# ZhuoQiuMcgill/ReinforcementLearning4MeshGeneration

Measured on AMD Instinct MI355X. Metric: env-steps/sec at N_envs=4096 per GPU, boundary() domain, 1 MI355X, higher is better.
Workload: dtype f64

## Files before the change

reinforcementlearning4meshgeneration_amd/csrc/meshenv_eval.h:

```cpp
#pragma once

#include "meshenv_quality.h"

namespace meshenv {

constexpr int kEvalWaves = 8;

struct EvalTallyArgs {
    int n, step;
    const double *reward;
    const uint8_t *done, *complete;
    const LastEpisode *last_ep;
    const int32_t *target, *offset;
    int32_t *count, *length, *seen;
    double *ret, *ret_raw;
    int32_t *short_envs;
    int32_t *ep_env, *ep_domain, *ep_step, *ep_length, *ep_flags, *ep_n_elem, *ep_archive;
    double *ep_return, *ep_return_raw, *ep_quality;
};

__global__ void __launch_bounds__(64) k_eval_begin(DevState S, EvalTallyArgs A)
{
    const int lane = lane_id(), env = blockIdx.x * 64 + lane;
    bool wants = false;
    if (env < A.n) {
        A.count[env] = 0;
        A.length[env] = 0;
        A.ret[env] = 0.0;
        A.ret_raw[env] = 0.0;
        A.seen[env] = A.last_ep ? A.last_ep[env].episodes : 0;
        wants = A.target[env] > 0;
    }
    const unsigned long long m = __ballot(wants);
    if (lane == 0 && m) atomicAdd(A.short_envs, (int)__popcll(m));
}

__global__ void __launch_bounds__(64 * kEvalWaves) k_eval_tally(DevState S, EvalTallyArgs A)
{
    __shared__ int s_slot[64];
    __shared__ unsigned long long s_rec, s_scored;
    const int lane = lane_id(), wave = uniform_i32(threadIdx.x >> 6);
    const int base = blockIdx.x * 64, env = base + lane;
    if (wave == 0) {
        const bool live = env < A.n;
        bool rec = false, archived = false, reached = false;
        int slot = 0;
        if (live) {
            const double r = A.reward[env];
            const int len = A.length[env] + 1;
            const double ret = A.ret[env] + (double)(float)r;
            const double raw = A.ret_raw[env] + r;
            const LastEpisode le = A.last_ep ? A.last_ep[env] : LastEpisode{0, 0, 0, 0};
            const int seen = A.seen[env];
            if (A.last_ep && le.episodes != seen) A.seen[env] = le.episodes;
            if (A.done[env]) {
                archived = A.last_ep && le.episodes != seen;
                const int cnt = A.count[env], tgt = A.target[env];
                if (cnt < tgt) {
                    rec = true;
                    slot = A.offset[env] + cnt;
                    A.ep_env[slot] = env;
                    A.ep_domain[slot] = S.scal[env].dom;
                    A.ep_step[slot] = A.step;
                    A.ep_length[slot] = len;
                    A.ep_return[slot] = ret;
                    A.ep_return_raw[slot] = raw;
                    A.ep_flags[slot] = (A.complete[env] ? 1 : 0) | (archived ? (le.flags & 2) : 0);
                    A.ep_n_elem[slot] = A.last_ep ? (archived ? le.n_elem : 0) : -1;
                    if (A.ep_archive) A.ep_archive[slot] = archived ? le.episodes : 0;
                    A.count[env] = cnt + 1;
                    reached = cnt + 1 == tgt;
                }
                A.length[env] = 0;
                A.ret[env] = 0.0;
                A.ret_raw[env] = 0.0;
            } else {
                A.length[env] = len;
                A.ret[env] = ret;
                A.ret_raw[env] = raw;
            }
        }
        s_slot[lane] = slot;
        const unsigned long long rec_mask = __ballot(rec), scored_mask = __ballot(rec && archived);
        const unsigned long long reached_mask = __ballot(reached);
        if (lane == 0 && reached_mask) atomicSub(A.short_envs, (int)__popcll(reached_mask));
        if (lane == 0) {
            s_rec = rec_mask;
            s_scored = scored_mask;
        }
    }
    if (!A.ep_quality) return;
    __syncthreads();
    const unsigned long long rec = s_rec, scored = s_scored;
    unsigned long long todo = ((unsigned long long)(unsigned)uniform_i32((int)(rec >> 32)) << 32) |
                              (unsigned)uniform_i32((int)(unsigned)rec);
    if (!todo) return;
    const DevCold cold = *S.cold;
    for (int k = 0; todo; k++) {
        const int l = __builtin_ctzll(todo);
        todo &= todo - 1;
        if (k % kEvalWaves != wave) continue;
        double *row = A.ep_quality + (size_t)uniform_i32(s_slot[l]) * 4 * kQualityDim;
        if ((scored >> l) & 1) env_quality(S, S.scal[base + l], cold, base + l, 1, nullptr, row, nullptr);
        else if (lane < 4 * kQualityDim) row[lane] = 0.0;
    }
}

}
```

reinforcementlearning4meshgeneration_amd/csrc/meshenv_hip.hip:

```cpp
#include "../../include/meshenv.h"
#include "../../include/meshenv_optim.h"

#include <hip/hip_runtime.h>
#include <link.h>

#include <cmath>
#include <cstdio>
#include <cstdlib>
#include <cstring>
#include <mutex>
#include <string>
#include <vector>

#include "meshenv_actor.h"
#include "meshenv_domgen.h"
#include "meshenv_kernels.h"
#include "meshenv_quality.h"
#include "meshenv_smooth.h"
#include "meshenv_samples.h"
#include "meshenv_fused.h"
#include "meshenv_policy.h"
#include "meshenv_gae.h"
#include "meshenv_eval.h"
#include "meshenv_replay.h"
// ... 410 lines not shown
    }
    CREATE_HIP(upload_atan_state());

    {
        int n_cu = 256;
        CREATE_HIP(hipDeviceGetAttribute(&n_cu, hipDeviceAttributeMultiprocessorCount, device));
        if (n_cu <= 0) n_cu = 256;
        h->n_cu = n_cu;
        int G = 1;
        const char *force = getenv("MESHENV_GROUP");
        int want = 1;
        if (force) want = atoi(force);
        else if (n_envs <= n_cu * 16) {
            int g = 1;
            while (g * 2 <= n_envs / n_cu && g * 2 <= 16) g *= 2;
            want = g >= 8 ? g : 1;
        }
        for (int g : {16, 8})
            if (g <= want && group_lds_bytes(cap, g) <= 150 * 1024) { G = g; break; }
        if (!force && (G < 8 || n_envs > n_cu * G)) G = 1;
        if (G == 1 && want == 16 && n_envs <= n_cu * 16 && group_lds_bytes(cap, 16) > 150 * 1024) {
            std::vector<int2> pack((size_t)n_envs);
            size_t worst = 0;
            for (int w0 = 0; w0 < n_envs; w0 += 16) {
                size_t off = 0;
                for (int e = w0; e < w0 + 16 && e < n_envs; e++) {
                    const int d = env_domain_host[e];
                    const int n0 = dom_offsets_host[d + 1] - dom_offsets_host[d];
                    const int cap_e = (n0 + 15) / 16 * 16;
                    pack[(size_t)e] = make_int2((int)off, cap_e);
                    off += lds_bytes_for(cap_e);
                }
                worst = off > worst ? off : worst;
            }
            worst = (worst + 31) / 32 * 32;
            if (worst + 16 * sizeof(Handoff) <= (size_t)kLdsCap) {
                G = 16;
                h->env_lds_host.swap(pack);
                h->ho_off = (int)worst;
            }
        }
        MeshEnvParams def;
        meshenv_default_params(&def);
        h->default_params = prm.radius == def.radius && prm.max_ref_angle == def.max_ref_angle && prm.key_lambda == def.key_lambda &&
                            prm.min_degree == def.min_degree && prm.max_degree == def.max_degree &&
                            prm.same_point_eps == def.same_point_eps && prm.ray_length == def.ray_length;
        if (!h->default_params) G = 1;
        if (!h->default_params) h->env_lds_host.clear();
        h->group = G;
        h->group_lds = h->env_lds_host.empty() ? group_lds_bytes(cap, G) : (size_t)h->ho_off + 16 * sizeof(Handoff);
        {
            const char *lz = getenv("MESHENV_LAZY");
            const bool lazy = lz ? atoi(lz) != 0 : n_envs >= 8192;
            const char *lt = getenv("MESHENV_LIGHT");
            const bool light = lt ? atoi(lt) != 0 : (lazy && n_envs >= 16384);
            h->stage_bits = (lazy ? 2 : 0) | (light ? 4 : 0);
        }
        if (G > 1 && h->group_lds > 64 * 1024) {
            const bool ragged = !h->env_lds_host.empty();
            const void *fn = ragged ? (const void *)k_step_group<16, true, true>
                             : G == 16 ? (const void *)k_step_group<16, true> : (const void *)k_step_group<8, true>;
            if (!ragged && cap <= 64) fn = G == 16 ? (const void *)k_step_group<16, true, false, true> : (const void *)k_step_group<8, true, false, true>;
            CREATE_HIP(hipFuncSetAttribute(fn, hipFuncAttributeMaxDynamicSharedMemorySize, kLdsCap));
        }
    }

    DevState &S = h->S;
    S.n_domains = n_domains;
    S.n_envs = n_envs;
    S.prm.radius = prm.radius;
    S.prm.max_ref_angle = prm.max_ref_angle;
    S.prm.w0 = prm.key_lambda;
    S.prm.w1 = 1 - prm.key_lambda;
    S.prm.min_degree = prm.min_degree;
    S.prm.max_degree = prm.max_degree;
    S.prm.same_eps = prm.same_point_eps;
    S.prm.ray_length = prm.ray_length;
    S.prm.fail_limit = prm.fail_limit;
    S.prm.log_cap = prm.log_capacity;

    const int total_dom = dom_offsets_host[n_domains];
    h->dom_off_host.assign(dom_offsets_host, dom_offsets_host + n_domains + 1);
    h->env_dom_host.assign(env_domain_host, env_domain_host + n_envs);
    const size_t total_env = (size_t)n_envs * (size_t)cap;
    S.cap = cap;

    double2 *d_dom_xy = nullptr;
    DevCold &K = h->cold;
    std::memset(&K, 0, sizeof(K));
    CREATE_TRY(dev_alloc(h, &S.dom, (size_t)n_domains));
    CREATE_TRY(dev_alloc(h, &d_dom_xy, (size_t)total_dom));
    CREATE_TRY(dev_alloc(h, &K.dom_key, (size_t)total_dom));
    CREATE_TRY(dev_alloc(h, &K.dom_stamp, (size_t)total_dom));
    CREATE_TRY(dev_alloc(h, &K.dom_obs, (size_t)n_domains * kObsDim));
    CREATE_TRY(dev_alloc(h, &S.ring_xy, total_env));
    CREATE_TRY(dev_alloc(h, &S.ring_id, total_env));
    CREATE_TRY(dev_alloc(h, &S.ring_key, total_env));
    CREATE_TRY(dev_alloc(h, &S.ring_stamp, total_env));
    CREATE_TRY(dev_alloc(h, &S.scal, (size_t)n_envs));
    CREATE_TRY(dev_alloc(h, &S.cnt, (size_t)n_envs));
    CREATE_TRY(dev_alloc(h, &S.obs_cache, (size_t)n_envs * kObsDim));
    if (!h->env_lds_host.empty()) {
        CREATE_TRY(dev_alloc(h, &h->env_lds, (size_t)n_envs));
        CREATE_HIP(hipMemcpy(h->env_lds, h->env_lds_host.data(), sizeof(int2) * (size_t)n_envs, hipMemcpyHostToDevice));
    }
    if (prm.log_capacity > 0) {
        CREATE_TRY(dev_alloc(h, &K.log_quads, (size_t)n_envs * 2 * prm.log_capacity * 4));
        CREATE_TRY(dev_alloc(h, &K.log_vxy, (size_t)n_envs * 2 * prm.log_capacity));
        CREATE_TRY(dev_alloc(h, &K.last_ep, (size_t)n_envs));
        CREATE_HIP(hipMemsetAsync(K.last_ep, 0, sizeof(LastEpisode) * (size_t)n_envs, h->stream));
    }
    K.dom_xy = d_dom_xy;
    {
        DevCold *cold_dev = nullptr;
        CREATE_TRY(dev_alloc(h, &cold_dev, (size_t)1));
        CREATE_HIP(hipMemcpy(cold_dev, &K, sizeof(DevCold), hipMemcpyHostToDevice));
        S.cold = cold_dev;
    }
#ifdef MESHENV_STAMPS
    CREATE_TRY(dev_alloc(h, &S.dbg, (size_t)n_envs * 16));
#endif

    std::vector<EnvScalars> sc((size_t)n_envs);
    std::memset(sc.data(), 0, sc.size() * sizeof(EnvScalars));
    for (int e = 0; e < n_envs; e++) sc[e].dom = env_domain_host[e];

    if (!gen) {
        std::vector<DomConst> dc((size_t)n_domains);
        std::memset(dc.data(), 0, dc.size() * sizeof(DomConst));
        for (int d = 0; d < n_domains; d++) {
            dc[d].orig_area = dom_consts_host[3 * d];
            dc[d].min_area = dom_consts_host[3 * d + 1] * dom_consts_host[3 * d + 1];
            dc[d].crit_area = dom_consts_host[3 * d + 2] * dom_consts_host[3 * d + 2];
            dc[d].off = dom_offsets_host[d];
            dc[d].n0 = dom_offsets_host[d + 1] - dom_offsets_host[d];
            dc[d].ref = -1;
        }
        CREATE_HIP(hipMemcpy(S.dom, dc.data(), sizeof(DomConst) * (size_t)n_domains, hipMemcpyHostToDevice));
        CREATE_HIP(hipMemcpy(d_dom_xy, dom_xy_host, sizeof(double2) * (size_t)total_dom, hipMemcpyHostToDevice));
    } else {
        int32_t *d_off = nullptr;
        int *d_err = nullptr;
        CREATE_TRY(dev_alloc(h, &d_off, (size_t)n_domains + 1));
        CREATE_TRY(dev_alloc(h, &d_err, (size_t)1));
        CREATE_HIP(hipMemcpy(d_off, dom_offsets_host, sizeof(int32_t) * ((size_t)n_domains + 1), hipMemcpyHostToDevice));
        CREATE_HIP(hipMemset(d_err, 0, sizeof(int)));
        if (gen->density_mode)
            hipLaunchKernelGGL(k_gen_rings_density, dim3(n_domains), dim3(64), 0, h->stream, *gen, n_domains, (const int32_t *)d_off, d_dom_xy, d_err);
        else
            hipLaunchKernelGGL(k_gen_rings, dim3(n_domains), dim3(64), 0, h->stream, *gen, n_domains, (const int32_t *)d_off, d_dom_xy, d_err);
        CREATE_HIP(hipGetLastError());
        hipLaunchKernelGGL(k_dom_consts, dim3(n_domains), dim3(64), sizeof(double2) * (size_t)max_ring, h->stream, n_domains,
                           (const int32_t *)d_off, (const double2 *)d_dom_xy, S.dom);
        CREATE_HIP(hipGetLastError());
        int err = 0;
        CREATE_HIP(hipMemcpy(&err, d_err, sizeof(int), hipMemcpyDeviceToHost));
        if (err) {
            g_create_error = "meshenv_create_random: a ring could not be generated on the device (fewer than 5 distinct pixels, or a length mismatch between the two passes)";
            meshenv_destroy(h);
            return MESHENV_E_STATE;
        }
    }
    CREATE_HIP(hipMemcpy(S.scal, sc.data(), sizeof(EnvScalars) * (size_t)n_envs, hipMemcpyHostToDevice));
    CREATE_HIP(hipMemset(S.ring_xy, 0, sizeof(double2) * total_env));
    CREATE_HIP(hipMemset(S.ring_id, 0, sizeof(int32_t) * total_env));
    CREATE_HIP(hipMemset(S.ring_key, 0, sizeof(double) * total_env));
    CREATE_HIP(hipMemset(S.ring_stamp, 0, sizeof(int32_t) * total_env));

    hipLaunchKernelGGL(k_init_domains, dim3(n_domains), dim3(64), lds, h->stream, S, cap);
    CREATE_HIP(hipGetLastError());
    hipLaunchKernelGGL(k_reset, dim3(n_envs), dim3(64), lds, h->stream, S, cap, (const uint8_t *)nullptr, (float *)nullptr, 1, 0ULL,
                       0, (int32_t *)nullptr, (int32_t *)nullptr);
    CREATE_HIP(hipGetLastError());
    CREATE_HIP(hipStreamSynchronize(h->stream));
#undef CREATE_TRY
#undef CREATE_HIP
    *out = h;
    return MESHENV_OK;
}

extern "C" {

int meshenv_create(int device, int n_domains, const int32_t *dom_offsets_host, const double *dom_xy_host,
                   const double *dom_consts_host, int n_envs, const int32_t *env_domain_host,
                   const MeshEnvParams *params, void *stream, MeshEnv **out)
{
    return create_impl(device, n_domains, dom_offsets_host, dom_xy_host, dom_consts_host, n_envs, env_domain_host, params,
                       stream, nullptr, out);
}

static void edge_direction(double dx, double dy, bool integer, double *cs)
{
    volatile double ny = (integer && dy == 0) ? 0.0 : -dy, x = dx;
    const double theta = -std::atan2(ny, x);
    volatile double angle = std::copysign(1.0, theta) >= 0 ? theta : 2 * 3.141592653589793 + theta;
    cs[0] = std::cos(angle);
    cs[1] = std::sin(angle);
}

static int create_random_impl(const char *fn, int device, int n_envs, GenParams gp, const uint64_t *seeds_host,
                              const MeshEnvParams *params, void *stream, MeshEnv **out, uint8_t *raises_host)
{
    int ndev = 0;
    if (hipGetDeviceCount(&ndev) != hipSuccess || ndev <= 0) {
        g_create_error = std::string(fn) + ": no HIP device available (this library has no CPU fallback)";
        return MESHENV_E_HIP;
    }
    if (device < 0 || device >= ndev) return fail_arg(nullptr, "meshenv_create_random: device index out of range");
    std::vector<int32_t> offs((size_t)n_envs + 1, 0), env_dom((size_t)n_envs);
    DeviceGuard guard(device);
    if (guard.err != hipSuccess) { g_create_error = std::string(fn) + ": hipSetDevice failed"; return MESHENV_E_HIP; }
    int32_t *d_cnt = nullptr;
    int *d_err = nullptr;
    unsigned long long *d_seeds = nullptr;
    double2 *d_tab = nullptr;
    unsigned char *d_raises = nullptr;
    auto cleanup = [&]() {
        if (d_cnt) (void)hipFree(d_cnt);
        if (d_err) (void)hipFree(d_err);
        if (d_seeds) (void)hipFree(d_seeds);
        if (d_tab) (void)hipFree(d_tab);
        if (d_raises) (void)hipFree(d_raises);
    };
    bool ok = hipMalloc((void **)&d_cnt, sizeof(int32_t) * (size_t)n_envs) == hipSuccess &&
              hipMalloc((void **)&d_err, sizeof(int)) == hipSuccess && hipMemset(d_err, 0, sizeof(int)) == hipSuccess;
    if (ok && seeds_host) {
        ok = hipMalloc((void **)&d_seeds, sizeof(unsigned long long) * (size_t)n_envs) == hipSuccess &&
             hipMemcpy(d_seeds, seeds_host, sizeof(unsigned long long) * (size_t)n_envs, hipMemcpyHostToDevice) == hipSuccess;
        gp.seeds = d_seeds;
    }
    if (ok && gp.density_mode) {
        const int R = (int)std::ceil(4 * gp.ave_radius) + 1, W = 2 * R + 1;
        std::vector<double> tab((size_t)W * W * 2);
        for (int dx = -R; dx <= R; dx++)
            for (int dy = -R; dy <= R; dy++) edge_direction((double)dx, (double)dy, true, &tab[((size_t)(dx + R) * W + (dy + R)) * 2]);
        ok = hipMalloc((void **)&d_tab, sizeof(double2) * (size_t)W * W) == hipSuccess &&
             hipMemcpy(d_tab, tab.data(), sizeof(double) * tab.size(), hipMemcpyHostToDevice) == hipSuccess &&
             hipMalloc((void **)&d_raises, (size_t)n_envs) == hipSuccess && hipMemset(d_raises, 0, (size_t)n_envs) == hipSuccess;
        gp.dir_tab = d_tab;
        gp.dir_r = R;
        gp.raises = d_raises;
    }
    int err = 0;
    if (ok) {
        if (gp.density_mode) hipLaunchKernelGGL(k_gen_count_density, dim3(n_envs), dim3(64), 0, (hipStream_t)stream, gp, n_envs, d_cnt, d_err);
        else hipLaunchKernelGGL(k_gen_count, dim3(n_envs), dim3(64), 0, (hipStream_t)stream, gp, n_envs, d_cnt, d_err);
        ok = hipGetLastError() == hipSuccess && hipStreamSynchronize((hipStream_t)stream) == hipSuccess &&
             hipMemcpy(offs.data() + 1, d_cnt, sizeof(int32_t) * (size_t)n_envs, hipMemcpyDeviceToHost) == hipSuccess &&
             hipMemcpy(&err, d_err, sizeof(int), hipMemcpyDeviceToHost) == hipSuccess;
    }
// ... 427 lines not shown
    const size_t lds = smooth_lds_bytes(h->cap, log_cap), lds_front = smooth_front_lds_bytes(h->cap, log_cap);
    if (lds > 160 * 1024 || (!interior && lds_front > 160 * 1024) || h->cap + log_cap > 65535)
        return fail_arg(h, "meshenv_smooth: ring stride + log_capacity too large for the smoother's LDS (16 B per ring slot + 60 B per logged vertex; front smoother 51 B per vertex)");
    MESHENV_ON_DEVICE(h);
    {
        const int rc = ensure_smooth_state(h);
        if (rc != MESHENV_OK) return rc;
    }
    int32_t *sw = sweeps_dev ? sweeps_dev : h->smooth_sweeps;
    if (!interior) return launch_full_smoothing(h, mask_dev, iteration, is_static, sw, diff_dev, obs_dev);
    const dim3 grid(h->n_envs), block(64);
    hipLaunchKernelGGL(k_smooth_interior, grid, block, lds, h->stream, h->S, h->cap, which, mask_dev, (const int32_t *)nullptr,
                       iteration, sw, diff_dev);
    HIP_TRY(h, hipGetLastError());
    if (which) return MESHENV_OK;
    hipLaunchKernelGGL(k_rebuild_candidates<0>, grid, block, h->lds, h->stream, h->S, h->cap, mask_dev, sw, h->pend, h->pend_obs,
                       (float *)nullptr, libm_ref(h));
    HIP_TRY(h, hipGetLastError());
    h->reselect_pending = true;
    return MESHENV_OK;
}

int meshenv_smooth_final(MeshEnv *h, int which, const uint8_t *mask_dev, int iteration, double lr_1, double lr_2,
                         int32_t *sweeps_dev, double *diff_dev)
{
    if (!h || (which != 0 && which != 1)) return MESHENV_E_ARG;
    if (iteration < 0) return fail_arg(h, "meshenv_smooth_final: iteration must be >= 0");
    const int log_cap = h->S.prm.log_cap;
    if (log_cap <= 0) {
        h->err = "meshenv_smooth_final: handle was created with log_capacity = 0 (the mesh graph is rebuilt from the element log)";
        return MESHENV_E_STATE;
    }
    const size_t lds = smooth_final_lds_bytes(h->cap, log_cap);
    if (lds > 160 * 1024 || h->cap + log_cap > 65535)
        return fail_arg(h, "meshenv_smooth_final: ring stride + log_capacity too large for the smoother's LDS (51 B per vertex)");
    MESHENV_ON_DEVICE(h);
    if (!h->smooth_final_ready) {
        HIP_TRY(h, hipFuncSetAttribute((const void *)k_smooth_final, hipFuncAttributeMaxDynamicSharedMemorySize, 160 * 1024));
        h->smooth_final_ready = true;
    }
    hipLaunchKernelGGL(k_smooth_final, dim3(h->n_envs), dim3(64), lds, h->stream, h->S, h->cap, which, mask_dev, iteration, lr_1,
                       lr_2, sweeps_dev, diff_dev);
    HIP_TRY(h, hipGetLastError());
    return MESHENV_OK;
}

int meshenv_get_not_valid(MeshEnv *h, int env, double *xy_host, int cap_points, int32_t *count)
{
    if (!h || !count) return MESHENV_E_ARG;
    if (env < 0 || env >= h->n_envs) {
        h->err = "meshenv_get_not_valid: env out of range";
        return MESHENV_E_RANGE;
    }
    *count = 0;
    if (!h->move_ready) return MESHENV_OK;
    MESHENV_ON_DEVICE(h);
    HIP_TRY(h, hipStreamSynchronize(h->stream));
    int32_t n = 0;
    HIP_TRY(h, hipMemcpy(&n, h->nv_count + env, sizeof(n), hipMemcpyDeviceToHost));
    *count = n;
    if (xy_host && n > 0) {
        const int m = n < cap_points ? n : cap_points;
        HIP_TRY(h, hipMemcpy(xy_host, h->nv_xy + (size_t)env * h->cap, sizeof(double2) * (size_t)m, hipMemcpyDeviceToHost));
    }
    return MESHENV_OK;
}

int meshenv_get_not_valid_ids(MeshEnv *h, int env, int32_t *ids_host, int cap_ids, int32_t *count, int32_t *last_host)
{
    if (!h || !count) return MESHENV_E_ARG;
    if (env < 0 || env >= h->n_envs) {
        h->err = "meshenv_get_not_valid_ids: env out of range";
        return MESHENV_E_RANGE;
    }
    *count = 0;
    if (last_host) last_host[0] = last_host[1] = last_host[2] = last_host[3] = 0;
    if (!h->move_ready) return MESHENV_OK;
    MESHENV_ON_DEVICE(h);
    HIP_TRY(h, hipStreamSynchronize(h->stream));
    int32_t n = 0, meta[kNvMeta];
    HIP_TRY(h, hipMemcpy(&n, h->nv_count + env, sizeof(n), hipMemcpyDeviceToHost));
    HIP_TRY(h, hipMemcpy(meta, h->nv_meta + (size_t)env * kNvMeta, sizeof(meta), hipMemcpyDeviceToHost));
    EnvScalars s;
    HIP_TRY(h, hipMemcpy(&s, h->S.scal + env, sizeof(s), hipMemcpyDeviceToHost));
    const int n0 = h->dom_off_host[s.dom + 1] - h->dom_off_host[s.dom];
    auto gid = [n0](int32_t g) { return (g & kNewBit) ? n0 + (g & ~kNewBit) : g; };
    *count = n;
    if (ids_host && n > 0) {
        const int m = n < cap_ids ? n : cap_ids;
        HIP_TRY(h, hipMemcpy(ids_host, h->nv_gid + (size_t)env * h->cap, sizeof(int32_t) * (size_t)m, hipMemcpyDeviceToHost));
        for (int i = 0; i < m; i++) ids_host[i] = gid(ids_host[i]);
    }
    if (last_host) {
        last_host[0] = gid(meta[1]); last_host[1] = gid(meta[2]); last_host[2] = meta[3];
        last_host[3] = meta[4] == meta[0] ? 1 : 0;
    }
    return MESHENV_OK;
}

static int launch_step(MeshEnv *h, int n_steps, const float *actions_dev, float *obs_dev, double *reward_dev,
                       uint8_t *done_dev, uint8_t *complete_dev, float *terminal_obs_dev, int auto_reset)
{
    if (!h) return MESHENV_E_ARG;
    if (!actions_dev || !obs_dev || !reward_dev || !done_dev || !complete_dev) return fail_arg(h, "meshenv_step: null device pointer");
    if (n_steps <= 0) return fail_arg(h, "meshenv_rollout: n_steps must be positive");
    if (n_steps > 1 && h->reselect_pending) {
        h->err = "meshenv_rollout: the first step after meshenv_smooth must be a meshenv_step (it commits the re-selection "
                 "the candidate rebuild parked, include/meshenv.h)";
        return MESHENV_E_STATE;
    }
    MESHENV_ON_DEVICE(h);
    const size_t slot = (size_t)(h->ev_count % MESHENV_TIMING_POOL);
    const long long pos = h->timing > 0 ? (h->launch_count++ % (2LL * h->timing)) : -1;
    if (pos == 0) HIP_TRY(h, hipEventRecord(h->ev[2 * slot], h->stream));
    if (n_steps == 1 && h->group > 1 && !h->front_moved) {
        const int G = h->group;
        const dim3 grid((h->n_envs + G - 1) / G), block(64 * G);
        GroupArgs A;
        A.S = h->S;
        A.outs.obs_out = obs_dev; A.outs.reward = reward_dev; A.outs.done = done_dev; A.outs.complete = complete_dev;
        A.outs.term_obs = terminal_obs_dev;
        A.actions = actions_dev;
        A.step0 = (unsigned long long)h->steps_done;
        A.cap = h->cap;
        A.auto_reset = auto_reset;
        A.env_lds = h->env_lds;
        A.ho_off = h->ho_off;
        A.pad = 0;
        if (h->env_lds) hipLaunchKernelGGL((k_step_group<16, true, true>), grid, block, h->group_lds, h->stream, A);
        else if (h->cap <= 64 && G == 16) hipLaunchKernelGGL((k_step_group<16, true, false, true>), grid, block, h->group_lds, h->stream, A);
        else if (h->cap <= 64) hipLaunchKernelGGL((k_step_group<8, true, false, true>), grid, block, h->group_lds, h->stream, A);
        else if (G == 16) hipLaunchKernelGGL((k_step_group<16, true>), grid, block, h->group_lds, h->stream, A);
        else hipLaunchKernelGGL((k_step_group<8, true>), grid, block, h->group_lds, h->stream, A);
    } else {
        const dim3 grid(h->n_envs), block(64);
#define MESHENV_LAUNCH_STEP(MULTI, DEF)                                                                                      \
    do {                                                                                                                     \
        KStepArgs ka;                                                                                                        \
        ka.S = h->S; ka.cap = h->cap; ka.n_steps = n_steps; ka.actions = actions_dev; ka.obs_out = obs_dev;                  \
        ka.reward = reward_dev; ka.done = done_dev; ka.complete = complete_dev; ka.term_obs = terminal_obs_dev;              \
        ka.auto_reset = auto_reset; ka.step0 = (unsigned long long)h->steps_done;                                            \
        if (h->front_moved) hipLaunchKernelGGL((k_step<MULTI, DEF, true>), grid, block, h->lds, h->stream, ka);              \
        else if (DEF && !MULTI && (h->stage_bits & 2) && h->cap <= 64)                                                       \
            hipLaunchKernelGGL((k_step<false, DEF, false, DEF, DEF>), grid, block, h->lds, h->stream, ka);                   \
        else if (DEF && !MULTI && (h->stage_bits & 2))                                                                       \
            hipLaunchKernelGGL((k_step<false, DEF, false, false, DEF>), grid, block, h->lds, h->stream, ka);                 \
        else if (DEF && h->cap <= 64) hipLaunchKernelGGL((k_step<MULTI, DEF, false, DEF>), grid, block, h->lds, h->stream, ka); \
        else hipLaunchKernelGGL((k_step<MULTI, DEF>), grid, block, h->lds, h->stream, ka);                                   \
    } while (0)
        if (n_steps == 1) {
            auto_reset = (auto_reset ? 1 : 0) | h->stage_bits;
            if (h->default_params) MESHENV_LAUNCH_STEP(false, true);
            else MESHENV_LAUNCH_STEP(false, false);
        } else {
            if (h->default_params) MESHENV_LAUNCH_STEP(true, true);
            else MESHENV_LAUNCH_STEP(true, false);
        }
#undef MESHENV_LAUNCH_STEP
    }
    HIP_TRY(h, hipGetLastError());
    if (h->reselect_pending) {
        hipLaunchKernelGGL(k_apply_reselect, dim3(h->n_envs), dim3(64), 0, h->stream, h->S, h->pend, h->pend_obs, obs_dev);
        HIP_TRY(h, hipGetLastError());
        h->reselect_pending = false;
    }
    h->steps_done += (uint64_t)n_steps;
    if (pos >= 0 && pos == h->timing - 1) {
        HIP_TRY(h, hipEventRecord(h->ev[2 * slot + 1], h->stream));
        h->ev_count += 1;
    }
    return MESHENV_OK;
}

int meshenv_step(MeshEnv *h, const float *actions_dev, float *obs_dev, double *reward_dev, uint8_t *done_dev,
                 uint8_t *complete_dev, float *terminal_obs_dev, int auto_reset)
{
    return launch_step(h, 1, actions_dev, obs_dev, reward_dev, done_dev, complete_dev, terminal_obs_dev, auto_reset);
}

int meshenv_rollout(MeshEnv *h, int n_steps, const float *actions_dev, float *obs_dev, double *reward_dev,
                    uint8_t *done_dev, uint8_t *complete_dev, int auto_reset)
{
    return launch_step(h, n_steps, actions_dev, obs_dev, reward_dev, done_dev, complete_dev, nullptr, auto_reset);
}

__global__ void k_status(DevState S, uint8_t *out)
{
    const int e = blockIdx.x * blockDim.x + threadIdx.x;
    if (e < S.n_envs) out[e] = (uint8_t)(S.scal[e].status & 3);
}

int meshenv_get_status(MeshEnv *h, uint8_t *status_dev)
{
    if (!h || !status_dev) return MESHENV_E_ARG;
    MESHENV_ON_DEVICE(h);
    hipLaunchKernelGGL(k_status, dim3((h->n_envs + 255) / 256), dim3(256), 0, h->stream, h->S, status_dev);
    HIP_TRY(h, hipGetLastError());
    return MESHENV_OK;
}

int meshenv_get_state(MeshEnv *h, int env, int32_t *ring_ids_host, double *ring_xy_host, double *cand_key_host,
                      int32_t *cand_stamp_host, int32_t *scalars_host, double *fscalars_host)
{
    if (!h) return MESHENV_E_ARG;
    if (env < 0 || env >= h->n_envs) {
        h->err = "meshenv_get_state: env out of range";
        return MESHENV_E_RANGE;
    }
    MESHENV_ON_DEVICE(h);
    HIP_TRY(h, hipStreamSynchronize(h->stream));
    EnvScalars s;
    HIP_TRY(h, hipMemcpy(&s, h->S.scal + env, sizeof(s), hipMemcpyDeviceToHost));
    const size_t off = (size_t)env * (size_t)h->cap;
    const int n0 = h->dom_off_host[s.dom + 1] - h->dom_off_host[s.dom];
    const int n = s.n;
    if (ring_ids_host) {
        HIP_TRY(h, hipMemcpy(ring_ids_host, h->S.ring_id + off, sizeof(int32_t) * n, hipMemcpyDeviceToHost));
        for (int i = 0; i < n; i++)
            if (ring_ids_host[i] & kNewBit) ring_ids_host[i] = n0 + (ring_ids_host[i] & ~kNewBit);
    }
    if (ring_xy_host) HIP_TRY(h, hipMemcpy(ring_xy_host, h->S.ring_xy + off, sizeof(double2) * n, hipMemcpyDeviceToHost));
    if (cand_stamp_host || cand_key_host) {
        std::vector<int32_t> st((size_t)n);
        std::vector<double> ky((size_t)n);
        HIP_TRY(h, hipMemcpy(st.data(), h->S.ring_stamp + off, sizeof(int32_t) * n, hipMemcpyDeviceToHost));
        HIP_TRY(h, hipMemcpy(ky.data(), h->S.ring_key + off, sizeof(double) * n, hipMemcpyDeviceToHost));
        for (int i = 0; i < n; i++) {
            if (cand_stamp_host) cand_stamp_host[i] = st[i];
            if (cand_key_host) cand_key_host[i] = st[i] == kNotCand ? NAN : ky[i];
        }
    }
    if (scalars_host) {
        scalars_host[0] = s.n;
        scalars_host[1] = s.ref;
        scalars_host[2] = s.n_elem;
        scalars_host[3] = s.failed;
        scalars_host[4] = n0 + s.n_new;
        scalars_host[5] = s.status & 3;
        scalars_host[6] = s.dom;
        scalars_host[7] = n0;
    }
    if (fscalars_host) {
        fscalars_host[0] = s.area;
        fscalars_host[1] = s.bl;
    }
    return MESHENV_OK;
}

static int fetch_elements(MeshEnv *h, const char *fn, int which, int env, int32_t *quads_host, int cap_elems,
                          double *vertex_xy_host, int cap_verts, int32_t *n_elem, int32_t *n_vert, int32_t *flags,
                          int32_t *episodes)
{
    if (!h || !n_elem || !n_vert) return MESHENV_E_ARG;
    if (env < 0 || env >= h->n_envs) {
        h->err = std::string(fn) + ": env out of range";
        return MESHENV_E_RANGE;
    }
    const int cap = h->S.prm.log_cap;
    if (cap <= 0) {
        h->err = std::string(fn) + ": handle was created with log_capacity = 0";
        return MESHENV_E_STATE;
    }
    MESHENV_ON_DEVICE(h);
    HIP_TRY(h, hipStreamSynchronize(h->stream));
    EnvScalars s;
    HIP_TRY(h, hipMemcpy(&s, h->S.scal + env, sizeof(s), hipMemcpyDeviceToHost));
    int half = (s.status >> 4) & 1, ne = s.n_elem, nnew = s.n_new;
    if (which) {
        LastEpisode le;
        HIP_TRY(h, hipMemcpy(&le, h->cold.last_ep + env, sizeof(le), hipMemcpyDeviceToHost));
        half ^= 1; ne = le.n_elem; nnew = le.n_new;
        if (flags) *flags = le.flags;
        if (episodes) *episodes = le.episodes;
    }
    const int d = s.dom;
    const int n0 = h->dom_off_host[d + 1] - h->dom_off_host[d];
    ne = ne < cap ? ne : cap;
    nnew = nnew < cap ? nnew : cap;
    if (ne > cap_elems) ne = cap_elems;
    int nv = n0 + nnew;
    if (nv > cap_verts) nv = cap_verts;
    const size_t base = ((size_t)env * 2 + half) * cap;
    if (quads_host && ne > 0) {
        HIP_TRY(h, hipMemcpy(quads_host, h->cold.log_quads + base * 4, sizeof(int32_t) * 4 * (size_t)ne, hipMemcpyDeviceToHost));
        for (int i = 0; i < 4 * ne; i++)
            if (quads_host[i] & kNewBit) quads_host[i] = n0 + (quads_host[i] & ~kNewBit);
    }
    if (vertex_xy_host && nv > 0) {
        const int first = nv < n0 ? nv : n0;
        HIP_TRY(h, hipMemcpy(vertex_xy_host, h->cold.dom_xy + h->dom_off_host[d], sizeof(double2) * (size_t)first, hipMemcpyDeviceToHost));
        if (nv > n0)
            HIP_TRY(h, hipMemcpy(vertex_xy_host + 2 * (size_t)n0, h->cold.log_vxy + base, sizeof(double2) * (size_t)(nv - n0), hipMemcpyDeviceToHost));
    }
    *n_elem = ne;
    *n_vert = nv;
    return MESHENV_OK;
}

int meshenv_get_elements(MeshEnv *h, int env, int32_t *quads_host, int cap_elems, double *vertex_xy_host,
                         int cap_verts, int32_t *n_elem, int32_t *n_vert)
{
    return fetch_elements(h, "meshenv_get_elements", 0, env, quads_host, cap_elems, vertex_xy_host, cap_verts, n_elem,
                          n_vert, nullptr, nullptr);
}

int meshenv_get_last_episode(MeshEnv *h, int env, int32_t *quads_host, int cap_elems, double *vertex_xy_host,
                             int cap_verts, int32_t *n_elem, int32_t *n_vert, int32_t *flags, int32_t *episodes)
{
    return fetch_elements(h, "meshenv_get_last_episode", 1, env, quads_host, cap_elems, vertex_xy_host, cap_verts,
                          n_elem, n_vert, flags, episodes);
}

int meshenv_element_quality(MeshEnv *h, int which, double *elem_dev, double *stats_dev, int32_t *count_dev)
{
    if (!h || (which != 0 && which != 1)) return MESHENV_E_ARG;
    if (h->S.prm.log_cap <= 0) {
        h->err = "meshenv_element_quality: handle was created with log_capacity = 0";
        return MESHENV_E_STATE;
    }
    MESHENV_ON_DEVICE(h);
    hipLaunchKernelGGL(k_element_quality, dim3(h->n_envs), dim3(64), 0, h->stream, h->S, which, elem_dev, stats_dev,
                       count_dev);
    HIP_TRY(h, hipGetLastError());
    return MESHENV_OK;
}

int meshenv_quad_quality(MeshEnv *h, int n, const double *quad_xy_dev, int index, double *out_dev)
{
    if (!h || n < 0 || (n > 0 && (!quad_xy_dev || !out_dev))) return MESHENV_E_ARG;
    if (!(index == 0 || index == 1 || index == 3 || index == 4 || index == 5))
        return fail_arg(h, "meshenv_quad_quality: index must be 0, 1, 3, 4 or 5 (2 and 6 add the boundary term of the extraction "
                           "step: that value is the step's reward)");
    if (n == 0) return MESHENV_OK;
    MESHENV_ON_DEVICE(h);
    hipLaunchKernelGGL(k_quad_quality, dim3((n + 63) / 64), dim3(64), 0, h->stream, n,
                       reinterpret_cast<const double2 *>(quad_xy_dev), index, out_dev);
    HIP_TRY(h, hipGetLastError());
    return MESHENV_OK;
}

int meshenv_counters(MeshEnv *h, uint64_t *out_host)
{
    if (!h || !out_host) return MESHENV_E_ARG;
    MESHENV_ON_DEVICE(h);
    HIP_TRY(h, hipStreamSynchronize(h->stream));
    std::vector<EnvCounters> c((size_t)h->n_envs);
    std::vector<EnvScalars> sc((size_t)h->n_envs);
    HIP_TRY(h, hipMemcpy(c.data(), h->S.cnt, sizeof(EnvCounters) * (size_t)h->n_envs, hipMemcpyDeviceToHost));
    HIP_TRY(h, hipMemcpy(sc.data(), h->S.scal, sizeof(EnvScalars) * (size_t)h->n_envs, hipMemcpyDeviceToHost));
    uint64_t a = h->steps_done * (uint64_t)h->n_envs, b = 0, s = 0, sv = 0;
    for (int e = 0; e < h->n_envs; e++) {
        const EnvCounters &k = c[(size_t)e];
        b += k.valid;
        s += k.sum_n + (uint64_t)sc[(size_t)e].n * (h->steps_done - k.last_change);
        sv += k.sum_n_valid;
    }
    out_host[0] = a;
    out_host[1] = b;
    out_host[2] = s;
    out_host[3] = sv;
    return MESHENV_OK;
}

#ifdef MESHENV_STAMPS
int meshenv_debug_raw_counters(MeshEnv *h, uint64_t *out_host)
{
    if (!h || !out_host) return MESHENV_E_ARG;
    HIP_TRY(h, hipStreamSynchronize(h->stream));
    HIP_TRY(h, hipMemcpy(out_host, h->S.cnt, sizeof(EnvCounters) * (size_t)h->n_envs, hipMemcpyDeviceToHost));
    return MESHENV_OK;
}
int meshenv_debug_stamps(MeshEnv *h, uint64_t *out_host)
{
    if (!h || !out_host) return MESHENV_E_ARG;
    HIP_TRY(h, hipStreamSynchronize(h->stream));
    HIP_TRY(h, hipMemcpy(out_host, h->S.dbg, sizeof(uint64_t) * 16 * (size_t)h->n_envs, hipMemcpyDeviceToHost));
    return MESHENV_OK;
}
#endif

__global__ void k_selftest(int what, int n, const double *in, double *out, int libm_exact)
{
    const int i = blockIdx.x * blockDim.x + threadIdx.x;
    if (i >= n) return;
    if (what == 0) out[i] = round4_py(in[i]);
    else if (what == 1) out[i] = round4_np(in[i]);
    else if (what == 2) out[i] = cw(mkp(in[6 * i], in[6 * i + 1]), mkp(in[6 * i + 2], in[6 * i + 3]), mkp(in[6 * i + 4], in[6 * i + 5]));
    else if (what == 3) out[i] = is_cross(mkp(in[8 * i], in[8 * i + 1]), mkp(in[8 * i + 2], in[8 * i + 3]), mkp(in[8 * i + 4], in[8 * i + 5]),
                                          mkp(in[8 * i + 6], in[8 * i + 7])) ? 1.0 : 0.0;
    else if (what == 4) out[i] = (sin_rounds_to_zero(in[2 * i], in[2 * i + 1]) ? 1.0 : 0.0) + (sin_rounds_to_zero_exact(in[2 * i], in[2 * i + 1]) ? 2.0 : 0.0);
    else if (what == 5) out[i] = (double)round4_npf((float)in[i]);
    else if (what == 6) out[i] = dist(mkp(in[4 * i], in[4 * i + 1]), mkp(in[4 * i + 2], in[4 * i + 3]));
    else if (what == 7) out[i] = (sqrt_pos(in[i]) == sqrt(in[i])) ? 1.0 : 0.0;
    else if (what == 8) {
        bool ne;
        const double f = cw_fast(in[2 * i], in[2 * i + 1], ne);
        const double e = cw_exact(in[2 * i], in[2 * i + 1]);
        out[i] = ne ? 1.0 : ((f == e && signbit(f) == signbit(e)) ? 0.0 : 2.0);
    } else if (what == 9 || what == 10) {
        const double *q = in + 9 * (size_t)i;
        FrontState f;
        f.coord = nullptr; f.adj = nullptr; f.deg = nullptr; f.ringu = nullptr; f.n = 0; f.n0 = 0; f.raised = 0; f.tab = nullptr; f.exact = libm_exact != 0;
        const P2 v = mkp(q[1], q[2]), a = mkp(q[3], q[4]), b = mkp(q[5], q[6]);
        const int which = (int)q[0];
        P2 r;
        if (which == 0) r = middle_vertex(f, v, a, b, q[7]);
        else if (which == 1) r = side_vertex(f, v, a, b, q[7], q[8], false);
        else if (which == 2) r = indention_vertex(f, v, a, b, q[7], q[8], false);
        else {
            const double2 e = estimate_4th_vertex(make_double2(v.x, v.y), make_double2(a.x, a.y), make_double2(b.x, b.y), q[7], q[8] >= 0, q[8]);
            r = mkp(e.x, e.y);
        }
        out[i] = f.raised ? __builtin_nan("") : (what == 9 ? r.x : r.y);
    } else if (what == 11) out[i] = pow2_glibc(in[i]);
    else if (what == 12) out[i] = cw_exact(in[2 * i], in[2 * i + 1]);
    else if (what == 13) {
        bool ok;
        const double t = atan2_glibc(in[2 * i], in[2 * i + 1], g_atan_cij, ok);
        out[i] = ok ? t : __builtin_nan("");
    } else if (what == 14) out[i] = atan2_cr(in[2 * i], in[2 * i + 1]);
    else if (what == 15) out[i] = sincos_small_nc(in[i]).s;
    else if (what == 16) out[i] = sincos_small_nc(in[i]).c;
    else if (what == 17) {
        const double *q = in + 7 * (size_t)i;
        const P2 ref = mkp(q[0], q[1]);
        const double tl = q[4];
        const double ux = (ref.x + q[2]) - ref.x, uy = (ref.y + q[3]) - ref.y;
        const P2 v = mkp(q[5], ref.y - 1), b = mkp(q[6], ref.y + 1);
        const double W = slab_half_width(tl);
        const double slab_lo = ref.x - W, slab_hi = ref.x + W;
        double s;
        out[i] = (slab_keeps(slab_lo, slab_hi, v.x, b.x) ? 1.0 : 0.0) + (bisector_hits(ref, ux, uy, v, b, s) ? 2.0 : 0.0) +
                 (dist(ref, v) < tl ? 4.0 : 0.0);
    } else if (what == 18) {
        const double *q = in + 7 * (size_t)i;
        const P2 p = mkp(q[0], q[1]), vi = mkp(q[2], q[3]), vm = mkp(q[4], q[5]), far = mkp(q[6], q[1]);
        out[i] = (pip_filter_usable(fabs(q[6] - p.x)) && pip_edge_clear(p, vi, vm) ? 1.0 : 0.0) + (straddle(p, far, vi, vm) && straddle(vi, vm, p, far) ? 2.0 : 0.0);
    } else if (what == 19) {
        const double *q = in + 9 * (size_t)i;
        P2 m[4];
        for (int k = 0; k < 4; k++) m[k] = mkp(q[2 * k], q[2 * k + 1]);
        double rec[kQualityDim];
        element_quality(m, rec);
        double r = __builtin_nan("");
        for (int k = 0; k < kQualityDim; k++) r = q[8] == (double)k ? rec[k] : r;
        out[i] = r;
    }
}

int meshenv_selftest(int device, int what, int n, int in_per_item, const double *in_host, double *out_host)
{
    if (n <= 0 || !in_host || !out_host || in_per_item <= 0) return MESHENV_E_ARG;
// ... 1329 lines not shown
```

reinforcementlearning4meshgeneration_amd/csrc/meshenv_kernels.h:

```cpp
#pragma once

#include "meshenv_geom.h"
#include "meshenv_libm.h"
#include "meshenv_state.h"

namespace meshenv {

constexpr int kStNoReference = 1;
constexpr int kStLogOverflow = 2;
constexpr int kStRm1Bad = 4, kStRp1Bad = 8;
constexpr int kNvMeta = 8;
constexpr int kStLogHalf = 16;

#ifdef MESHENV_STAMPS
#define MESHENV_STAMP(c, k) do { if ((c).lane == 0) (c).sc->stamps[k] = __builtin_amdgcn_s_memrealtime(); } while (0)
#else
#define MESHENV_STAMP(c, k) do { } while (0)
#endif

struct Scratch {
    double2 q[4];
    double ang[4];
    double tmp[16];
    double tmp2[8];
    float robs[18];
    int ipad[2];
    unsigned long long red[6];
#ifdef MESHENV_STAMPS
    unsigned long long stamps[16];
#endif
};

struct Ctx {
    double2 *xy;
    double *key;
    int32_t *stamp;
    int32_t *id;
    double *ang_ord;
    int32_t *list;
    Scratch *sc;
    int lane, env;
    size_t base;
    int n, ref, n_elem, failed, n_new, counter, status, dom;
    double bl, area, ct, st;
    bool ring_dirty;
    bool tie = false;
    float obs;
};

__device__ __forceinline__ P2 ldp(const Ctx &c, int i)
{
    const double2 v = c.xy[i];
    return mkp(v.x, v.y);
}

__device__ __forceinline__ void wave_sync()
{
    __builtin_amdgcn_fence(__ATOMIC_ACQ_REL, "wavefront");
    __builtin_amdgcn_wave_barrier();
}

__device__ __forceinline__ int spin_until_nonzero(volatile int *w)
{
    int v = *w;
    for (int it = 0; v == 0 && it < (1 << 22); it++) {
        __builtin_amdgcn_s_sleep(1);
        v = *w;
    }
    return v;
}

__device__ __forceinline__ int wrapi(int i, int n)
{
    const unsigned a = (unsigned)i, b = (unsigned)(i + n), c = (unsigned)(i - n);
    const unsigned m = a < b ? a : b;
    return (int)(m < c ? m : c);
}

__host__ __device__ __forceinline__ size_t lds_bytes_for(int cap)
{
    return ((size_t)cap * (sizeof(double2) + 2 * sizeof(double) + 3 * sizeof(int32_t)) + sizeof(Scratch) + 64 + 15) / 16 * 16;
}

__device__ __forceinline__ void carve_lds(Ctx &c, void *smem, int cap)
{
    c.xy = (double2 *)smem;
    c.key = (double *)(c.xy + cap);
    c.ang_ord = c.key + cap;
    c.stamp = (int32_t *)(c.ang_ord + cap);
    c.id = c.stamp + cap;
    c.list = c.id + cap;
    c.sc = (Scratch *)(c.list + cap);
}


struct EnvLoad {
    EnvScalars s;
    double2 v_xy, w_xy;
    double v_key, w_key;
    int v_id, v_st, w_id, w_st;
    float obs;
};

__device__ __forceinline__ EnvLoad load_env_issue(const DevState &S, int env, const bool with_keys = true)
{
    EnvLoad L;
    const int lane = lane_id();
    const size_t base = (size_t)env * S.cap;
    L.s = S.scal[env];
    const int first = S.cap < 64 ? S.cap : 64;
    const double2 *gxy = S.ring_xy + base;
    const int32_t *gid = S.ring_id + base;
    const double *gkey = S.ring_key + base;
    const int32_t *gst = S.ring_stamp + base;
    const unsigned ul = (unsigned)lane;
    L.v_xy = make_double2(0, 0); L.w_xy = make_double2(0, 0);
    L.v_key = 0; L.w_key = 0;
    L.v_id = 0; L.v_st = kNotCand; L.w_id = 0; L.w_st = kNotCand;
    if (lane < first) {
        L.v_xy = gxy[ul];
        L.v_id = gid[ul];
        if (with_keys) {
            L.v_key = gkey[ul];
            L.v_st = gst[ul];
        }
    }
    const bool second = S.cap > 64 && (int)(64u + ul) < S.cap;
    if (second) {
        L.w_xy = gxy[64u + ul];
        L.w_id = gid[64u + ul];
        if (with_keys) {
            L.w_key = gkey[64u + ul];
            L.w_st = gst[64u + ul];
        }
    }
    L.obs = lane < kObsDim ? S.obs_cache[(size_t)env * kObsDim + lane] : 0.0f;
    return L;
}

__device__ __forceinline__ void load_env_commit(Ctx &c, const DevState &S, int env, const EnvLoad &L, const bool with_keys = true,
                                                const int lds_cap = 0)
{
    const int lane = lane_id();
    c.lane = lane;
    c.env = env;
    c.base = (size_t)env * S.cap;
    const EnvScalars &s = L.s;
    const int lcap = lds_cap > 0 ? lds_cap : S.cap;
    const int first = lcap < 64 ? lcap : 64;
    const double2 *gxy = S.ring_xy + c.base;
    const int32_t *gid = S.ring_id + c.base;
    const double *gkey = S.ring_key + c.base;
    const int32_t *gst = S.ring_stamp + c.base;
    const unsigned ul = (unsigned)lane;
    const bool second = lcap > 64 && (int)(64u + ul) < lcap;
    c.obs = L.obs;
    c.n = uniform_i32(s.n); c.ref = uniform_i32(s.ref); c.n_elem = uniform_i32(s.n_elem);
    c.failed = uniform_i32(s.failed); c.n_new = uniform_i32(s.n_new); c.counter = uniform_i32(s.counter);
    c.status = uniform_i32(s.status); c.dom = uniform_i32(s.dom);
    c.bl = uniform_f64(s.bl); c.area = uniform_f64(s.area); c.ct = uniform_f64(s.ct); c.st = uniform_f64(s.st);
    c.ring_dirty = false;
    if (lane < first) {
        c.xy[lane] = L.v_xy;
        c.id[lane] = L.v_id;
        if (with_keys) {
            c.key[lane] = L.v_key;
            c.stamp[lane] = L.v_st;
        }
    }
    if (second) {
        c.xy[64u + ul] = L.w_xy;
        c.id[64u + ul] = L.w_id;
        if (with_keys) {
            c.key[64u + ul] = L.w_key;
            c.stamp[64u + ul] = L.w_st;
        }
    }
    for (unsigned i = 128u + ul; i < (unsigned)c.n; i += 64u) {
        c.xy[i] = gxy[i];
        c.id[i] = gid[i];
        if (with_keys) {
            c.key[i] = gkey[i];
            c.stamp[i] = gst[i];
        }
    }
    wave_sync();
}

__device__ __forceinline__ void load_env(Ctx &c, const DevState &S, int env, const bool with_keys = true, const int lds_cap = 0)
{
    const EnvLoad L = load_env_issue(S, env, with_keys);
    load_env_commit(c, S, env, L, with_keys, lds_cap);
}

__device__ __forceinline__ void load_keys(Ctx &c, const DevState &S)
{
    const double *gkey = S.ring_key + c.base;
    const int32_t *gst = S.ring_stamp + c.base;
    for (unsigned i = (unsigned)c.lane; i < (unsigned)c.n; i += 64u) {
        c.key[i] = gkey[i];
        c.stamp[i] = gst[i];
    }
    wave_sync();
}

__device__ __forceinline__ void store_ring(const Ctx &c, const DevState &S)
{
    double2 *gxy = S.ring_xy + c.base;
    int32_t *gid = S.ring_id + c.base;
    double *gkey = S.ring_key + c.base;
    int32_t *gst = S.ring_stamp + c.base;
    for (unsigned i = (unsigned)c.lane; i < (unsigned)c.n; i += 64u) {
        gxy[i] = c.xy[i];
        gid[i] = c.id[i];
        gkey[i] = c.key[i];
        gst[i] = c.stamp[i];
    }
}

__device__ __forceinline__ void store_env(Ctx &c, const DevState &S, bool ring_elsewhere = false)
{
    wave_sync();
    if (c.ring_dirty) {
        if (!ring_elsewhere) store_ring(c, S);
        if (c.lane < kObsDim) S.obs_cache[(size_t)c.env * kObsDim + c.lane] = c.obs;
    }
    if (c.lane == 0) {
        if (c.ring_dirty) {
            EnvScalars s;
            s.n = c.n; s.ref = c.ref; s.n_elem = c.n_elem; s.failed = c.failed; s.n_new = c.n_new;
            s.counter = c.counter; s.status = c.status; s.dom = c.dom; s.bl = c.bl; s.area = c.area;
            s.ct = c.ct; s.st = c.st;
            S.scal[c.env] = s;
        } else {
            int2 *fs = reinterpret_cast<int2 *>(&S.scal[c.env].failed);
            *fs = make_int2(c.failed, c.status);
        }
    }
}


__device__ __forceinline__ int select_reference(const Ctx &c)
{
    double bk = kInf;
    int bs = kNotCand, bi = -1;
    for (int i = c.lane; i < c.n; i += 64) {
        const int st = c.stamp[i];
        if (st != kNotCand) {
            const double k = c.key[i];
            if (k < bk || (k == bk && st > bs)) { bk = k; bs = st; bi = i; }
        }
    }
    const double kmin = wave_min_f64(bk);
    if (!(kmin < kInf)) return -1;
    const int smax = wave_max_i32(bk == kmin ? bs : kNotCand);
    const unsigned long long hit = __ballot(bk == kmin && bs == smax);
    return lane_i32(bi, (int)__ffsll((long long)hit) - 1);
}

__device__ __forceinline__ int select_reference_nv(const Ctx &c, const double2 *nv, int n_nv)
{
    double bk = kInf;
    int bs = kNotCand, bi = -1;
    for (int i = c.lane; i < c.n; i += 64) {
        const int st = c.stamp[i];
        if (st != kNotCand) {
            const P2 v = ldp(c, i);
            bool listed = false;
            for (int k = 0; k < n_nv; k++) listed = listed || dist(mkp(nv[k].x, nv[k].y), v) < 0.001;
            const double k = c.key[i];
            if (!listed && (k < bk || (k == bk && st > bs))) { bk = k; bs = st; bi = i; }
        }
    }
    const double kmin = wave_min_f64(bk);
    if (!(kmin < kInf)) return -1;
    const int smax = wave_max_i32(bk == kmin ? bs : kNotCand);
    const unsigned long long hit = __ballot(bk == kmin && bs == smax);
    return lane_i32(bi, (int)__ffsll((long long)hit) - 1);
}

__device__ __forceinline__ void key_angle_terms(const Ctx &c, int index, int which, double &cc, double &dd)
{
    const int n = c.n, o = which + 1;
    cw_terms(ldp(c, index), ldp(c, wrapi(index + o, n)), ldp(c, wrapi(index - o, n)), cc, dd);
}

__device__ __forceinline__ bool key_from_angles(const Params &p, double a0, double a1, double &out)
{
    if (a0 >= p.max_ref_angle || a0 == 0.0) return false;
    double sum_angle = 0.0;
    sum_angle += a0 * p.w0;
    sum_angle += a1 * p.w1;
    out = sum_angle * (180.0 / kPi);
    return true;
}


struct BqArgs {
    int mode;
    int a, b;
    double ang0, ang1;
    double q_ang0, q_ang2;
    double half01, half23;
    double mesh_area;
    double b_reward;
    bool skip;
};

__device__ __forceinline__ double dist_lr(const LibmRef lr, P2 a, P2 b)
{
    if (lr.tab == nullptr || !lr.exact) return dist(a, b);
    return sqrt_pos(pow2_nc(a.x - b.x) + pow2_nc(a.y - b.y));
}

__device__ __forceinline__ double slab_half_width(double target_length)
{
    return target_length * (1 + 1e-9) + 1e-9;
}
// ... 988 lines not shown
        double m_d = kInf;
        int carry = 0;
        const int bqi = bqa;
        const int w1 = wrapi(bqi + 1, n), w2 = wrapi(bqi + 2, n), w3 = wrapi(bqi - 1, n), w4 = wrapi(bqi - 2, n);
        const P2 add_v = ldp(c, bqi);
        const DistThr dst_thr = dist_thr(dst);
        for (int base = 0; base < n; base += 64) {
            const int i = base + lane;
            bool near = false;
            if (i < n && !(i == bqi || i == w1 || i == w2 || i == w3 || i == w4)) near = dist_lt(add_v, ldp(c, i), dst_thr);
            const unsigned long long m = __ballot(near);
            bool added = false;
            if (near) {
                const unsigned long long zeros_below = ~m & ((1ULL << lane) - 1ULL);
                if (zeros_below != 0ULL) {
                    const int pz = 63 - __clzll((long long)zeros_below);
                    added = ((lane - pz - 1) & 1) == 0;
                } else {
                    added = (lane & 1) == carry;
                }
            }
            if (added) {
                const double dd = seg_point_distance(ldp(c, wrapi(i + 1, n)), ldp(c, i), add_v);
                m_d = dd < m_d ? dd : m_d;
            }
            carry = (int)((__ballot(added) >> 63) & 1ULL);
        }
        m_d = wave_min_f64(m_d);
        const double targt_len = dst / 2;
        const double mean_dist = bq_sum / 4;
        const double smoothness = (targt_len < mean_dist ? targt_len : mean_dist) / (targt_len > mean_dist ? targt_len : mean_dist);
        double q2 = 1.0;
        if (m_d < 1e299) q2 = (m_d < 0.5 * dst) ? m_d / (0.5 * dst) : 1.0;
        b_reward = cbrt(smoothness * q1 * q2);
    } else {
        const double targt_len = bq_d0;
        const double mean_dist = bq_sum5 / 5;
        const double smoothness = (targt_len < mean_dist ? targt_len : mean_dist) / (targt_len > mean_dist ? targt_len : mean_dist);
        b_reward = sqrt(q1 * smoothness);
    }
    const double quality = e_reward + 1 * (b_reward - 1);
    double reward = 0.0;
    reward += quality + speed;
    if (n <= 5) reward += 10.0;
    return reward;
}

__device__ __forceinline__ StepResult env_finish(Ctx &c, const Params &prm, const Decision &d)
{
    StepResult out;
    out.valid = d.ok != 0;
    int done = d.done, complete = d.no_reference ? 0 : 1;
    if (d.ok) {
        c.failed = 0;
    } else {
        c.failed += 1;
        if (c.failed >= prm.fail_limit) {
            done = 1;
            complete = 0;
        }
    }
    out.reward = d.reward;
    out.done = done;
    out.complete = complete;
    return out;
}

__device__ __forceinline__ StepResult env_step(Ctx &c, const DevState &S, float a0, float a1, float a2, const bool pre_reject)
{
    Decision d = env_check(c, S, a0, a1, a2, pre_reject);
    if (d.ok) env_apply(c, S, d);
    return env_finish(c, S.prm, d);
}


__global__ void __launch_bounds__(64) k_init_domains(DevState S, int cap)
{
    extern __shared__ double2 smem[];
    Ctx c;
    carve_lds(c, smem, cap);
    const int d = blockIdx.x;
    c.lane = lane_id();
    c.env = -1;
    c.base = 0;
    c.dom = d;
    const DomConst dc = S.dom[d];
    const DevCold cold = load_cold(S);
    const int doff = dc.off;
    c.n = dc.n0;
    c.area = dc.orig_area;
    c.status = 0;
    c.bl = 0.0; c.ct = 1.0; c.st = 0.0;
    c.obs = 0.0f;
    for (int i = c.lane; i < c.n; i += 64) {
        c.xy[i] = cold.dom_xy[doff + i];
        c.id[i] = i;
    }
    wave_sync();
    for (int i = c.lane; i < c.n; i += 64) {
        double cc, dd, k = 0.0;
        key_angle_terms(c, i, 0, cc, dd);
        const double a0 = cw_exact(cc, dd);
        key_angle_terms(c, i, 1, cc, dd);
        const double a1 = cw_exact(cc, dd);
        const bool ok = key_from_angles(S.prm, a0, a1, k);
        c.key[i] = k;
        c.stamp[i] = ok ? -i : kNotCand;
    }
    BqArgs bq;
    bq.skip = false;
    bq.mode = 0; bq.a = 0; bq.b = 0; bq.ang0 = 0; bq.ang1 = 0; bq.q_ang0 = 0; bq.q_ang2 = 0; bq.half01 = 0; bq.half23 = 0;
    find_next_state(c, S, bq);
    for (int i = c.lane; i < c.n; i += 64) {
        cold.dom_key[doff + i] = c.key[i];
        cold.dom_stamp[doff + i] = c.stamp[i];
    }
    if (c.lane < kObsDim) cold.dom_obs[(size_t)d * kObsDim + c.lane] = c.obs;
    if (c.lane == 0) {
        S.dom[d].ref = c.ref;
        S.dom[d].bl = c.bl;
        S.dom[d].ct = c.ct;
        S.dom[d].st = c.st;
    }
}

__global__ void __launch_bounds__(64) k_reset(DevState S, int cap, const uint8_t *mask, float *obs_out, int first,
                                               unsigned long long step_now, int is_static, int32_t *nv_count,
                                               int32_t *nv_meta)
{
    extern __shared__ double2 smem[];
    Ctx c;
    carve_lds(c, smem, cap);
    const int env = blockIdx.x;
    const bool doit = mask == nullptr || mask[env] != 0;
    c.lane = lane_id();
    if (!doit) {
        if (obs_out && c.lane < kObsDim) obs_out[(size_t)env * kObsDim + c.lane] = S.obs_cache[(size_t)env * kObsDim + c.lane];
        return;
    }
    c.env = env;
    c.base = (size_t)env * S.cap;
    c.dom = uniform_i32(S.scal[env].dom);
    if (first) {
        c.n = 0; c.n_elem = 0; c.n_new = 0; c.status = 0;
    } else {
        c.n = uniform_i32(S.scal[env].n);
        c.n_elem = uniform_i32(S.scal[env].n_elem);
        c.n_new = uniform_i32(S.scal[env].n_new);
        c.status = uniform_i32(S.scal[env].status);
    }
    const int n_old = c.n;
    reset_from_domain(c, S);
    if (is_static && c.lane == 1) c.obs = 0.0f;
    if (nv_count && c.lane == 0) {
        nv_count[env] = 0;
        nv_meta[(size_t)env * kNvMeta] += 1;
    }
    if (c.lane == 0) {
        EnvCounters z;
        if (first) {
            z.last_change = 0; z.valid = 0; z.sum_n = 0; z.sum_n_valid = 0;
        } else {
            z = S.cnt[env];
            z.sum_n += (unsigned long long)n_old * (step_now - z.last_change);
            z.last_change = step_now;
        }
        S.cnt[env] = z;
    }
    store_env(c, S);
    if (obs_out && c.lane < kObsDim) obs_out[(size_t)env * kObsDim + c.lane] = c.obs;
}

struct KStepArgs {
    DevState S;
    int cap, n_steps;
    const float *actions;
    float *obs_out;
    double *reward;
    uint8_t *done, *complete;
    float *term_obs;
    int auto_reset;
    unsigned long long step0;
};
template <bool kDefaultParams>
__device__ __forceinline__ KStepArgs late_kstep_args()
{
    typedef const __attribute__((address_space(4))) unsigned long long *qptr;
    qptr q = (qptr)__builtin_amdgcn_kernarg_segment_ptr();
    asm volatile("" : "+s"(q));
    static_assert(sizeof(KStepArgs) % 8 == 0, "whole quadwords");
    union { KStepArgs a; unsigned long long w[sizeof(KStepArgs) / 8]; } u;
#pragma unroll
    for (unsigned i = 0; i < sizeof(KStepArgs) / 8; i++) u.w[i] = q[i];
    if (kDefaultParams) apply_default_params(u.a.S.prm);
    return u.a;
}

#ifndef MESHENV_STEP_WAVES_PER_SIMD
#define MESHENV_STEP_WAVES_PER_SIMD 5
#endif
template <bool kMulti, bool kDefaultParams, bool kTie = false, bool kSmall = false, bool kPre = false>
__global__ void __launch_bounds__(64, MESHENV_STEP_WAVES_PER_SIMD)
k_step(const KStepArgs A)
{
    DevState S = A.S;
    const int cap = A.cap, n_steps = A.n_steps;
    if (kSmall) __builtin_assume(cap <= 64 && S.cap <= 64 && cap > 0 && S.cap > 0);
    const float *__restrict__ actions = A.actions;
    float *__restrict__ obs_out = A.obs_out;
    double *__restrict__ reward = A.reward;
    uint8_t *__restrict__ done = A.done, *__restrict__ complete = A.complete;
    float *__restrict__ term_obs = A.term_obs;
    (void)term_obs;
    int auto_reset = A.auto_reset;
    const unsigned long long step0 = A.step0;
    extern __shared__ double2 smem[];
    if (kDefaultParams) apply_default_params(S.prm);
    Ctx c;
    c.tie = kTie;
    carve_lds(c, smem, cap);
    const int env = blockIdx.x;
    const int E = S.n_envs;
    const float *a = actions + (size_t)env * 3;
    float a0 = a[0], a1 = a[1], a2 = a[2];
#ifdef MESHENV_STAMPS
    const unsigned long long stamp_t0 = __builtin_amdgcn_s_memrealtime();
    const unsigned long long stamp_c0 = __builtin_amdgcn_s_memtime();
#endif
    if (!kMulti && (auto_reset & 2)) {
        const EnvScalars s0 = S.scal[env];
        const int lane0 = lane_id();
        const float ob = lane0 < kObsDim ? S.obs_cache[(size_t)env * kObsDim + lane0] : 0.0f;
        const int st0 = uniform_i32(s0.status), failed0 = uniform_i32(s0.failed) + 1, ne0 = uniform_i32(s0.n_elem);
        const bool memo = (a0 <= -0.5f && (st0 & kStRm1Bad) != 0) || (a0 >= 0.5f && (st0 & kStRp1Bad) != 0);
        if (memo && uniform_i32(s0.ref) >= 0 && uniform_i32(s0.n) > 5 && failed0 < S.prm.fail_limit) {
            const double rw = ne0 ? -1.0 / ne0 : -1.0;
            if (lane0 < kObsDim) obs_out[(size_t)env * kObsDim + lane0] = ob;
            if (S.msg && lane0 < 21)
                S.msg[(size_t)env * 21 + lane0] = lane0 < kObsDim ? ob : (lane0 == 18 ? (float)rw : (lane0 == 19 ? 0.0f : 1.0f));
            if (lane0 == 0) {
                reward[env] = rw;
                done[env] = 0;
                complete[env] = 1;
                S.scal[env].failed = failed0;
            }
            return;
        }
    }
    const bool light = !kMulti && (auto_reset & 4) != 0;
    auto_reset &= 1;
#ifndef MESHENV_STAMPS
    EnvCounters cnt0;
    cnt0.last_change = 0; cnt0.valid = 0; cnt0.sum_n = 0; cnt0.sum_n_valid = 0;
    if (kMulti) cnt0 = S.cnt[env];
#endif
    if (light) load_env(c, S, env, false);
    else load_env(c, S, env);
    if (kSmall) __builtin_assume(c.n <= 64 && c.n >= 0);
#ifdef MESHENV_STAMPS
    const unsigned long long stamp_t1 = __builtin_amdgcn_s_memrealtime();
    if (c.lane < 16) c.sc->stamps[c.lane] = 0;
    wave_sync();
#endif
#ifdef MESHENV_STAMPS
    unsigned long long st_valid = 0;
#else
    EnvCounters k = cnt0;
    bool k_dirty = false;
#endif
    double last_reward = 0.0;
    int last_done = 0, last_complete = 0;
    const int T = kMulti ? n_steps : 1;
    for (int t = 0; t < T; t++) {
        if (kMulti) {
            asm volatile("" : "+v"(c.lane));
        }
        if (kMulti && t > 0) {
            const float *at = actions + ((size_t)t * E + env) * 3;
            a0 = at[0]; a1 = at[1]; a2 = at[2];
        }
        if (kSmall) __builtin_assume(c.n <= 64 && c.n >= 0);
        const int n_before = c.n;
        Decision d = env_check(c, S, a0, a1, a2, kMulti || kPre);
        if (d.ok) {
            if (light) load_keys(c, S);
            env_apply(c, S, d);
        }
        const StepResult r = env_finish(c, S.prm, d);
#ifndef MESHENV_STAMPS
        if (!kMulti) {
            const KStepArgs L = late_kstep_args<kDefaultParams>();
            const bool l_auto = (L.auto_reset & 1) != 0;
            if (r.valid || (r.done && l_auto)) {
                k = L.S.cnt[env];
                const unsigned long long next = L.step0 + 1ULL;
                k.sum_n += (unsigned long long)n_before * (next - k.last_change);
                k.last_change = next;
                if (r.valid) { k.valid += 1ULL; k.sum_n_valid += (unsigned long long)n_before; }
                k_dirty = true;
            }
            if (c.lane == 0) {
                L.reward[env] = r.reward;
                L.done[env] = (uint8_t)r.done;
                L.complete[env] = (uint8_t)r.complete;
            }
            if (r.done) {
                if (L.term_obs && c.lane < kObsDim) L.term_obs[(size_t)env * kObsDim + c.lane] = c.obs;
                if (l_auto) reset_from_domain(c, L.S);
            }
            if (c.lane < kObsDim) L.obs_out[(size_t)env * kObsDim + c.lane] = c.obs;
            if (L.S.msg && c.lane < 21) {
                const float v = c.lane < kObsDim ? c.obs : (c.lane == 18 ? (float)r.reward : (c.lane == 19 ? (float)r.done : (float)r.complete));
                L.S.msg[(size_t)env * 21 + c.lane] = v;
            }
            store_env(c, L.S);
            if (k_dirty && c.lane == 0) L.S.cnt[env] = k;
            return;
        }
#endif
#ifdef MESHENV_STAMPS
        if (r.valid) st_valid += 1;
#else
        if (r.valid || (r.done && auto_reset)) {
            const unsigned long long next = step0 + (unsigned long long)t + 1ULL;
            k.sum_n += (unsigned long long)n_before * (next - k.last_change);
            k.last_change = next;
            if (r.valid) { k.valid += 1ULL; k.sum_n_valid += (unsigned long long)n_before; }
            k_dirty = true;
        }
#endif
        const size_t o = (size_t)t * E + env;
        if (c.lane == 0) {
            reward[o] = r.reward;
            done[o] = (uint8_t)r.done;
            complete[o] = (uint8_t)r.complete;
        }
        last_reward = r.reward; last_done = r.done; last_complete = r.complete;
        if (r.done) {
#ifndef MESHENV_STAMPS
            const KStepArgs L = late_kstep_args<kDefaultParams>();
            if (L.term_obs && c.lane < kObsDim) L.term_obs[(size_t)env * kObsDim + c.lane] = c.obs;
            if (L.auto_reset & 1) reset_from_domain(c, L.S);
#else
            if (term_obs && c.lane < kObsDim) term_obs[(size_t)env * kObsDim + c.lane] = c.obs;
            if (auto_reset) reset_from_domain(c, S);
#endif
        }
    }
#ifndef MESHENV_STAMPS
    {
        const KStepArgs L = late_kstep_args<kDefaultParams>();
        if (c.lane < kObsDim) L.obs_out[(size_t)env * kObsDim + c.lane] = c.obs;
        if (L.S.msg && c.lane < 21) {
            const float v = c.lane < kObsDim ? c.obs : (c.lane == 18 ? (float)last_reward : (c.lane == 19 ? (float)last_done : (float)last_complete));
            L.S.msg[(size_t)env * 21 + c.lane] = v;
        }
        store_env(c, L.S);
        if (k_dirty && c.lane == 0) L.S.cnt[env] = k;
        return;
    }
#endif
    if (c.lane < kObsDim) obs_out[(size_t)env * kObsDim + c.lane] = c.obs;
    if (S.msg && c.lane < 21) {
        const float v = c.lane < kObsDim ? c.obs : (c.lane == 18 ? (float)last_reward : (c.lane == 19 ? (float)last_done : (float)last_complete));
        S.msg[(size_t)env * 21 + c.lane] = v;
    }
    store_env(c, S);
#ifdef MESHENV_STAMPS
    if (c.lane == 0) {
        EnvCounters k;
        k.last_change = stamp_t0; k.valid = stamp_t1; k.sum_n = __builtin_amdgcn_s_memrealtime();
        k.sum_n_valid = st_valid | ((unsigned long long)(a0 <= -0.5f ? 1 : (a0 >= 0.5f ? 2 : 0)) << 8);
        S.cnt[env] = k;
    }
    if (c.lane == 0) c.sc->stamps[15] = __builtin_amdgcn_s_memtime() - stamp_c0;
    wave_sync();
    if (c.lane < 16) S.dbg[(size_t)env * 16 + c.lane] = c.sc->stamps[c.lane];
#else
    if (k_dirty && c.lane == 0) S.cnt[env] = k;
#endif
}


enum { kMoveOk = 0, kMoveNone = 1, kMoveRaises = 2, kMoveNeedsSmoothing = 3, kMoveSmoothRaises = 4 };

__host__ __device__ __forceinline__ size_t move_lds_bytes(int cap) { return lds_bytes_for(cap) + sizeof(double2) * (size_t)cap; }

__global__ void __launch_bounds__(64) k_move(DevState S, int cap, const double *__restrict__ points,
                                              const double *__restrict__ types, float *__restrict__ obs_out,
                                              uint8_t *__restrict__ done, uint8_t *__restrict__ complete,
                                              uint8_t *__restrict__ code, double2 *__restrict__ nv_xy,
                                              int32_t *__restrict__ nv_count, int32_t *__restrict__ nv_gid, const LibmRef lr)
{
    extern __shared__ double2 smem[];
    Ctx c;
    c.tie = true;
    carve_lds(c, smem, cap);
    double2 *nv = (double2 *)((char *)smem + lds_bytes_for(cap));
    const int env = blockIdx.x;
    const double mv_r = points[2 * (size_t)env], mv_a = points[2 * (size_t)env + 1], mv_type = types[env];
    int n_nv = uniform_i32(nv_count[env]);
    load_env(c, S, env);
    const int lane = c.lane;
    if (c.ref < 0 || c.n <= 5) {
        if (lane < kObsDim) obs_out[(size_t)env * kObsDim + lane] = c.obs;
        if (lane == 0) { done[env] = 0; complete[env] = 0; code[env] = (uint8_t)kMoveRaises; }
        return;
    }
    c.status &= ~(kStRm1Bad | kStRp1Bad);
    double2 *gnv = nv_xy + (size_t)env * cap;
    for (int k = lane; k < n_nv; k += 64) nv[k] = gnv[k];
    wave_sync();
    const double2 refpt = c.xy[c.ref];
    const int refgid = c.id[c.ref];
    Decision d = env_check(c, S, 0.0f, 0.0f, 0.0f, false, true, mv_r, mv_a, mv_type);
    if (d.ok) {
        env_apply(c, S, d, nullptr, true, nv, n_nv, lr);
        n_nv = 0;
    } else {
        bool listed = false;
        const int32_t *gids = nv_gid + (size_t)env * cap;
        for (int k = lane; k < n_nv; k += 64) listed = listed || gids[k] == refgid;
        if (__ballot(listed) == 0ULL) {
            if (lane == 0) {
                nv[n_nv] = refpt;
                gnv[n_nv] = refpt;
                nv_gid[(size_t)env * cap + n_nv] = refgid;
            }
            n_nv += 1;
        }
        wave_sync();
        BqArgs bq;
        bq.skip = false;
        bq.mode = 0; bq.a = 0; bq.b = 0; bq.ang0 = 0; bq.ang1 = 0; bq.q_ang0 = 0; bq.q_ang2 = 0; bq.half01 = 0; bq.half23 = 0;
        find_next_state(c, S, bq, true, nv, n_nv, lr);
        c.ring_dirty = true;
    }
    const bool ring_unchanged = !d.ok;
    const bool none = c.ref < 0;
    const int cd = none ? (c.n > 4 ? kMoveNeedsSmoothing : kMoveNone) : kMoveOk;
    if (lane < kObsDim) obs_out[(size_t)env * kObsDim + lane] = c.obs;
    if (lane == 0) {
        done[env] = (uint8_t)((d.done || cd == kMoveNeedsSmoothing) ? 1 : 0);
        complete[env] = (uint8_t)(c.n <= 4 ? 1 : 0);
        code[env] = (uint8_t)cd;
        nv_count[env] = n_nv;
    }
    store_env(c, S, ring_unchanged);
}


struct alignas(32) Handoff {
    int valid;
    int simd;
    int upd_done;
    int helper_done;
    int env, n, ref, n_elem, failed, n_new, counter, status, dom;
    int lds_off, lds_cap;
    int pad;
    double bl, area, ct, st;
    EnvCounters cnt0;
    Decision d;
};

__host__ __device__ __forceinline__ size_t group_lds_bytes(int cap, int G)
{
    return (size_t)G * (lds_bytes_for(cap) + sizeof(Handoff));
}

struct StepOuts {
    float *obs_out;
    double *reward;
    uint8_t *done;
    uint8_t *complete;
    float *term_obs;
};

struct GroupArgs {
    DevState S;
    StepOuts outs;
    const float *actions;
    unsigned long long step0;
    int cap;
    int auto_reset;
    const int2 *env_lds;
    int ho_off;
    int pad;
};

__device__ __forceinline__ StepOuts late_outs()
{
    typedef const __attribute__((address_space(4))) char *kptr;
    kptr ka = (kptr)__builtin_amdgcn_kernarg_segment_ptr();
    asm volatile("" : "+s"(ka));
    typedef const __attribute__((address_space(4))) unsigned long long *qptr;
    qptr q = (qptr)(ka + offsetof(GroupArgs, outs));
    static_assert(sizeof(StepOuts) == 5 * sizeof(unsigned long long), "StepOuts is five pointers");
    StepOuts o;
    o.obs_out = (float *)q[0];
    o.reward = (double *)q[1];
    o.done = (uint8_t *)q[2];
    o.complete = (uint8_t *)q[3];
    o.term_obs = (float *)q[4];
    return o;
}

__device__ __forceinline__ DevState late_state(const DevState &S)
{
    typedef const __attribute__((address_space(4))) unsigned long long *qptr;
    qptr q = (qptr)__builtin_amdgcn_kernarg_segment_ptr();
    asm volatile("" : "+s"(q));
    constexpr unsigned kWords = offsetof(DevState, prm) / 8;
    static_assert(offsetof(DevState, prm) % 8 == 0, "whole quadwords before prm");
    union { DevState s; unsigned long long w[sizeof(DevState) / 8]; } u;
    u.s = S;
#pragma unroll
    for (unsigned i = 0; i < kWords; i++) u.w[i] = q[i];
    return u.s;
}

__device__ __forceinline__ void finish_and_store(Ctx &c, const DevState &S_in, const Decision &d, const EnvCounters &cnt0,
                                                 int n_before, int auto_reset, unsigned long long step0,
                                                 volatile int *helper_done = nullptr, float *actor_row = nullptr,
                                                 const bool cnt_late = false)
{
    const StepResult r = env_finish(c, S_in.prm, d);
    const int env = c.env;
    const DevState S = late_state(S_in);
    const StepOuts o = late_outs();
    float *__restrict__ obs_out = o.obs_out;
    double *__restrict__ reward = o.reward;
    uint8_t *__restrict__ done = o.done;
    uint8_t *__restrict__ complete = o.complete;
    float *__restrict__ term_obs = o.term_obs;
    const bool has_helper = helper_done != nullptr;
    if (c.lane == 0) {
        if (!has_helper) reward[env] = r.reward;
        done[env] = (uint8_t)r.done;
        complete[env] = (uint8_t)r.complete;
    }
    if (r.done) {
        if (term_obs && c.lane < kObsDim) term_obs[(size_t)env * kObsDim + c.lane] = c.obs;
        if (auto_reset) {
            if (has_helper) {
                spin_until_nonzero(helper_done);
                wave_sync();
            }
            reset_from_domain(c, S);
        }
    }
    if (c.lane < kObsDim) obs_out[(size_t)env * kObsDim + c.lane] = c.obs;
    if (actor_row && c.lane < kObsDim) actor_row[(c.lane & 3) * 8 + (c.lane >> 2)] = c.obs;
    if (S.msg && c.lane < 21 && !(has_helper && c.lane == 18)) {
        const float v = c.lane < kObsDim ? c.obs : (c.lane == 18 ? (float)r.reward : (c.lane == 19 ? (float)r.done : (float)r.complete));
        S.msg[(size_t)env * 21 + c.lane] = v;
    }
    store_env(c, S, has_helper && !r.done);
    if ((r.valid || (r.done && auto_reset)) && c.lane == 0) {
        EnvCounters k = cnt_late ? S.cnt[env] : cnt0;
        k.sum_n += (unsigned long long)n_before * (step0 + 1ULL - k.last_change);
        k.last_change = step0 + 1ULL;
        if (r.valid) { k.valid += 1ULL; k.sum_n_valid += (unsigned long long)n_before; }
        S.cnt[env] = k;
    }
}

template <int G, bool kDefaultParams, bool kRagged = false, bool kSmall = false>
__device__ __forceinline__ void step_group_body(const GroupArgs &A, float *actor_in = nullptr)
{
    const int tid = (int)threadIdx.x;
    extern __shared__ double2 smem[];
    DevState S = A.S;
    const int cap = A.cap, auto_reset = A.auto_reset;
    if (kSmall) __builtin_assume(cap <= 64 && S.cap <= 64 && cap > 0 && S.cap > 0);
    const float *__restrict__ actions = A.actions;
    if (kDefaultParams) apply_default_params(S.prm);
    const int wave = uniform_i32(tid >> 6);
    const size_t env_bytes = lds_bytes_for(cap);
    Handoff *ho = (Handoff *)((char *)smem + (kRagged ? (size_t)A.ho_off : (size_t)G * env_bytes));
    const int env = blockIdx.x * G + wave;
    const bool active = env < S.n_envs;
    int pending = 0;
#ifdef MESHENV_STAMPS
    const unsigned long long dbg_t0 = __builtin_amdgcn_s_memrealtime();
#endif
    if (active) {
        Ctx c;
        int my_off = (int)((size_t)wave * env_bytes), my_cap = cap;
        if (kRagged) {
            const int2 e = A.env_lds[env];
            my_off = uniform_i32(e.x);
            my_cap = uniform_i32(e.y);
        }
        carve_lds(c, (char *)smem + my_off, my_cap);
        const float *a = actions + (size_t)env * 3;
        const float a0 = a[0], a1 = a[1], a2 = a[2];
        EnvCounters cnt0;
        cnt0.last_change = 0; cnt0.valid = 0; cnt0.sum_n = 0; cnt0.sum_n_valid = 0;
        constexpr bool kCntLate = true;
        load_env(c, S, env, true, kRagged ? my_cap : 0);
        if (kSmall) __builtin_assume(c.n <= 64 && c.n >= 0);
        const int n_before = c.n;
        Decision d = env_check(c, S, a0, a1, a2, false, false, 0.0, 0.0, 0.5, true);
        if (!d.ok) {
            finish_and_store(c, S, d, cnt0, n_before, auto_reset, A.step0, nullptr, actor_in ? actor_in + wave * 132 : nullptr, kCntLate);
        } else {
            pending = 1;
            if (c.lane == 0) {
                Handoff &h = ho[wave];
                h.env = env; h.n = c.n; h.ref = c.ref; h.n_elem = c.n_elem; h.failed = c.failed; h.n_new = c.n_new;
                h.counter = c.counter; h.status = c.status; h.dom = c.dom;
                if (kRagged) { h.lds_off = my_off; h.lds_cap = my_cap; }
                h.bl = c.bl; h.area = c.area; h.ct = c.ct; h.st = c.st;
                h.d = d;
                h.upd_done = 0;
                h.helper_done = 0;
            }
        }
    }
    if ((tid & 63) == 0) {
        ho[wave].valid = pending;
        ho[wave].simd = (int)__builtin_amdgcn_s_getreg((4 << 0) | (4 << 6) | (1 << 11));
    }
#ifdef MESHENV_STAMPS
    const unsigned long long dbg_t1 = __builtin_amdgcn_s_memrealtime();
#endif
    __syncthreads();
#ifdef MESHENV_STAMPS
    const unsigned long long dbg_t2 = __builtin_amdgcn_s_memrealtime();
    if (active && (tid & 63) == 0) {
        unsigned long long *o = S.dbg + (size_t)env * 16;
        o[0] = dbg_t0; o[1] = dbg_t1; o[2] = dbg_t2; o[3] = (unsigned long long)pending; o[4] = 0; o[5] = 0;
#ifdef MESHENV_DBG_P1SET
        {
            Ctx cs;
            carve_lds(cs, (char *)smem + (kRagged ? A.env_lds[env].x : (int)((size_t)wave * env_bytes)), kRagged ? A.env_lds[env].y : cap);
            o[4] = cs.sc->stamps[MESHENV_DBG_P1SET ? 4 : 1];
            o[5] = cs.sc->stamps[MESHENV_DBG_P1SET ? 5 : 2];
        }
#endif
        if (!pending) o[15] = 0;
    }
#endif

    const int dl = tid & 63;
    int hv = 0, hs = -1;
    if (dl < G) {
        hv = ho[dl].valid;
        hs = ho[dl].simd & 3;
    }
    const unsigned vmask = (unsigned)__ballot(hv != 0);
    const int m = __popc(vmask);
    if (m == 0) return;
    const unsigned sm0 = (unsigned)__ballot(hs == 0), sm1 = (unsigned)__ballot(hs == 1);
    const unsigned sm2 = (unsigned)__ballot(hs == 2), sm3 = (unsigned)__ballot(hs == 3);
    const unsigned wbit = 1u << wave;
    const int my_simd = (sm1 & wbit) ? 1 : (sm2 & wbit) ? 2 : (sm3 & wbit) ? 3 : 0;
    const unsigned mine = my_simd == 0 ? sm0 : my_simd == 1 ? sm1 : my_simd == 2 ? sm2 : sm3;
    const bool balanced = __popc(sm0) * 4 == G && __popc(sm1) * 4 == G && __popc(sm2) * 4 == G && __popc(sm3) * 4 == G;
    int src = -1, hsrc = -1;
#ifdef MESHENV_NO_HELPER
    const bool helpers = false;
#else
    const bool helpers = balanced && G >= 4 && 2 * m <= G && m <= 8;
#endif
    if (balanced && G >= 4) {
        const int r = __popc(mine & ((1u << wave) - 1u));
        const int j = r * 4 + my_simd;
        int k = j < m ? j : -1;
        if (helpers && j >= m) {
            const unsigned long long t_lo = G >= 16 ? 0x1111300011000010ULL : 0x1111210011000010ULL;
            const unsigned long long t_hi = 0x2222321133001220ULL;
            const unsigned hcw = (unsigned)(((m <= 4 ? t_lo : t_hi) >> (16 * ((m - 1) & 3))) & 0xffffULL);
            const int mains_here = (m + 3 - my_simd) >> 2;
            const int t = r - mains_here;
            const int here = (int)((hcw >> (4 * my_simd)) & 15u);
            const int below = my_simd == 0 ? 0 : (int)((hcw & 15u) + (my_simd > 1 ? ((hcw >> 4) & 15u) : 0u) + (my_simd > 2 ? ((hcw >> 8) & 15u) : 0u));
            if (t >= 0 && t < here) k = below + t;
        }
        if (k >= 0) {
            unsigned rest = vmask;
            for (int t = 0; t < k; t++) rest &= rest - 1u;
            const int which = __ffs((int)rest) - 1;
            if (j < m) src = which;
            else hsrc = which;
        }
    } else if (vmask & (1u << wave)) {
        src = wave;
    }
    if (src < 0 && hsrc < 0) return;

    if (hsrc >= 0) {
        Ctx c;
        Handoff &h = ho[hsrc];
        if (kRagged) carve_lds(c, (char *)smem + uniform_i32(h.lds_off), uniform_i32(h.lds_cap));
        else carve_lds(c, (char *)smem + (size_t)hsrc * env_bytes, cap);
        c.lane = tid & 63;
        Decision d = h.d;
        d.index = uniform_i32(d.index); d.new_vertex = uniform_i32(d.new_vertex);
        d.t0 = uniform_i32(d.t0); d.t1 = uniform_i32(d.t1);
        const int henv = uniform_i32(h.env);
        const double rew = reward_on_helper(c, S, d, uniform_i32(h.n), uniform_i32(h.dom), &h.upd_done);
        wave_sync();
        if (c.n > 5) {
            c.env = henv;
            c.base = (size_t)henv * S.cap;
            store_ring(c, late_state(S));
        }
        if (c.lane == 0) {
            *(volatile int *)&h.helper_done = 1;
            const StepOuts o = late_outs();
            o.reward[henv] = rew;
            if (S.msg) S.msg[(size_t)henv * 21 + 18] = (float)rew;
        }
        return;
    }

    Ctx c;
    Handoff &h = ho[src];
    if (kRagged) carve_lds(c, (char *)smem + uniform_i32(h.lds_off), uniform_i32(h.lds_cap));
    else carve_lds(c, (char *)smem + (size_t)src * env_bytes, cap);
    c.lane = tid & 63;
    c.env = uniform_i32(h.env);
    c.base = (size_t)c.env * S.cap;
    c.n = uniform_i32(h.n); c.ref = uniform_i32(h.ref); c.n_elem = uniform_i32(h.n_elem); c.failed = uniform_i32(h.failed);
    if (kSmall) __builtin_assume(c.n <= 64 && c.n >= 0);
    c.n_new = uniform_i32(h.n_new); c.counter = uniform_i32(h.counter); c.status = uniform_i32(h.status); c.dom = uniform_i32(h.dom);
    c.bl = uniform_f64(h.bl); c.area = uniform_f64(h.area); c.ct = uniform_f64(h.ct); c.st = uniform_f64(h.st);
    c.ring_dirty = false;
    c.obs = 0.0f;
    Decision d = h.d;
    d.index = uniform_i32(d.index); d.new_vertex = uniform_i32(d.new_vertex);
    d.mp0 = uniform_i32(d.mp0); d.mp1 = uniform_i32(d.mp1); d.mp2 = uniform_i32(d.mp2); d.mp3 = uniform_i32(d.mp3);
    d.p0 = uniform_i32(d.p0); d.p1 = uniform_i32(d.p1); d.p2 = uniform_i32(d.p2); d.p3 = uniform_i32(d.p3);
    d.t0 = uniform_i32(d.t0); d.t1 = uniform_i32(d.t1); d.lo = uniform_i32(d.lo); d.hi = uniform_i32(d.hi);
    d.ok = 1;
    const EnvCounters cnt0 = S.cnt[c.env];
    const int n_before = c.n;
    env_apply(c, S, d, helpers ? &h.upd_done : nullptr);
#ifdef MESHENV_STAMPS
    const unsigned long long dbg_t8 = __builtin_amdgcn_s_memrealtime();
#endif
    finish_and_store(c, S, d, cnt0, n_before, auto_reset, A.step0, helpers ? &h.helper_done : nullptr,
                     actor_in ? actor_in + src * 132 : nullptr);
#ifdef MESHENV_STAMPS
    if (c.lane == 0) {
        const unsigned long long t_end = __builtin_amdgcn_s_memrealtime();
        unsigned long long *o = S.dbg + (size_t)c.env * 16;
        o[6] = c.sc->stamps[6]; o[7] = dbg_t2; o[8] = dbg_t8;
        for (int k = 9; k <= 14; k++) o[k] = c.sc->stamps[k];
        o[15] = t_end;
        if (active) {
            unsigned long long *w = S.dbg + (size_t)env * 16;
            w[4] = t_end; w[5] = (unsigned long long)(src + 1);
        }
    }
#endif
}


template <int G, bool kDefaultParams, bool kRagged = false, bool kSmall = false>
__global__ void __launch_bounds__(64 * G)
k_step_group(GroupArgs A)
{
    step_group_body<G, kDefaultParams, kRagged, kSmall>(A);
}

}
```

reinforcementlearning4meshgeneration_amd/csrc/meshenv_quality.h:

```cpp
#pragma once

#include "meshenv_geom.h"
#include "meshenv_state.h"

namespace meshenv {

constexpr int kQualityDim = 8;

__device__ __forceinline__ double wave_max_f64(double v)
{
#define STEP(CTRL, MASK)                                        \
    {                                                           \
        const double ov = dpp_f64<CTRL, MASK>(-kInf, v);        \
        v = ov > v ? ov : v;                                    \
    }
    MESHENV_DPP_REDUCE(STEP)
#undef STEP
    return lane_f64(v, 63);
}

__device__ __forceinline__ double wave_sum_f64(double v)
{
#define STEP(CTRL, MASK) { v += dpp_f64<CTRL, MASK>(0.0, v); }
    MESHENV_DPP_REDUCE(STEP)
// ... 41 lines not shown
        const double x2x = (p2.x - p1.x) + (p3.x - p0.x), x2y = (p2.y - p1.y) + (p3.y - p0.y);
        const double x12x = (p0.x - p1.x) + (p2.x - p3.x), x12y = (p0.y - p1.y) + (p2.y - p3.y);
        const double len1 = sqrt(x1x * x1x + x1y * x1y), len2 = sqrt(x2x * x2x + x2y * x2y);
        q[4] = sqrt(x12x * x12x + x12y * x12y) / (len2 < len1 ? len2 : len1);
    }
    const double stretch = sqrt(2.0) * emin / (d1 > d0 ? d1 : d0);
    q[3] = stretch;
    q[5] = sqrt(stretch * (amin / amax));
    q[6] = 0.5 * e[0] * e[1] * sin(ang[0]) + 0.5 * e[2] * e[3] * sin(ang[2]);
    const double aspect = emin != 0 ? emax / emin : 0.001;
    q[7] = 1 / (aspect + err);
}

__device__ __forceinline__ void env_quality(const DevState &S, const EnvScalars &sc, const DevCold &cold, int env, int which,
                                            double *__restrict__ elem_out, double *__restrict__ stats_row,
                                            int32_t *__restrict__ count_out)
{
    const int lane = lane_id();
    const int cap = S.prm.log_cap;
    int half = (uniform_i32(sc.status) >> 4) & 1;
    int ne = uniform_i32(sc.n_elem);
    if (which) {
        ne = uniform_i32(cold.last_ep[env].n_elem);
        half ^= 1;
    }
    ne = ne < cap ? ne : cap;
    const int doff = uniform_i32(S.dom[uniform_i32(sc.dom)].off);
    const int4 *quads = reinterpret_cast<const int4 *>(cold.log_quads + ((size_t)env * 2 + half) * cap * 4);
    const double2 *vnew = cold.log_vxy + ((size_t)env * 2 + half) * cap;
    double mn[kQualityDim], mx[kQualityDim], s1[kQualityDim], s2[kQualityDim];
#pragma unroll
    for (int k = 0; k < kQualityDim; k++) { mn[k] = kInf; mx[k] = -kInf; s1[k] = 0; s2[k] = 0; }
    for (int i = lane; i < ne; i += 64) {
        const int4 g = quads[i];
        const int gid[4] = {g.x, g.y, g.z, g.w};
        P2 m[4];
        bool missing = false;
#pragma unroll
        for (int k = 0; k < 4; k++) {
            const int kn = gid[k] & ~kNewBit;
            const bool created = (gid[k] & kNewBit) != 0;
            const double kNaN = __builtin_nan("");
            missing = missing || (created && kn >= cap);
            const double2 v = created ? (kn < cap ? vnew[kn] : make_double2(kNaN, kNaN)) : cold.dom_xy[doff + gid[k]];
            m[k] = mkp(v.x, v.y);
        }
        double q[kQualityDim];
        element_quality(m, q);
#pragma unroll
        for (int k = 0; k < kQualityDim; k++) q[k] = missing ? __builtin_nan("") : q[k];
        if (elem_out) {
            double2 *dst = reinterpret_cast<double2 *>(elem_out + ((size_t)env * cap + i) * kQualityDim);
#pragma unroll
            for (int k = 0; k < 4; k++) dst[k] = make_double2(q[2 * k], q[2 * k + 1]);
        }
#pragma unroll
        for (int k = 0; k < kQualityDim; k++) {
            mn[k] = q[k] < mn[k] ? q[k] : mn[k];
            mx[k] = q[k] > mx[k] ? q[k] : mx[k];
            s1[k] += q[k];
            s2[k] += q[k] * q[k];
        }
    }
    if (count_out && lane == 0) *count_out = ne;
    if (stats_row) {
        double r = 0;
#pragma unroll
        for (int k = 0; k < kQualityDim; k++) {
            const double a = wave_min_f64(mn[k]), b = wave_sum_f64(s1[k]), c = wave_max_f64(mx[k]), d = wave_sum_f64(s2[k]);
            const double avg = ne ? b / ne : 0.0;
            const double var = ne ? d / ne - avg * avg : 0.0;
            const int j = lane - 4 * k;
            r = j == 0 ? (ne ? a : 0.0) : (j == 1 ? avg : (j == 2 ? (ne ? c : 0.0) : (j == 3 ? var : r)));
        }
        if (lane < 4 * kQualityDim) stats_row[lane] = r;
    }
}

__global__ void __launch_bounds__(64)
k_element_quality(DevState S, int which, double *__restrict__ elem_out, double *__restrict__ stats_out,
                  int32_t *__restrict__ count_out)
{
    const int env = blockIdx.x;
    const EnvScalars sc = S.scal[env];
    const DevCold cold = load_cold(S);
    env_quality(S, sc, cold, env, which, elem_out, stats_out ? stats_out + (size_t)env * 4 * kQualityDim : nullptr,
                count_out ? count_out + env : nullptr);
}

__device__ __forceinline__ double quad_quality_index(const P2 *m, int index)
{
    const double kPi = 3.141592653589793;
    double e[4], ang[4];
#pragma unroll
    for (int i = 0; i < 4; i++) {
        e[i] = dist(m[i], m[(i + 3) & 3]);
        ang[i] = cw(m[i], m[(i + 1) & 3], m[(i + 3) & 3]);
    }
    if (index == 0 || index == 3 || index == 4) {
        double q[kQualityDim];
        element_quality(m, q);
        return index == 0 ? q[7] : (index == 3 ? q[3] : q[5]);
    }
    const double area = 0.5 * e[0] * e[1] * sin(ang[0]) + 0.5 * e[2] * e[3] * sin(ang[2]);
    double q1 = 0.0;
    if (!(area <= 0)) {
        const double ra = sqrt(area);
        double product = 1.0;
#pragma unroll
        for (int i = 0; i < 4; i++) product *= (ra - e[i] > 0) ? e[i] / ra : 1.0 / (e[i] / ra);
        q1 = pow(product, 0.25);
    }
    double ap = 1.0;
#pragma unroll
    for (int i = 0; i < 4; i++) ap *= 1 - (fabs(ang[i] * (180.0 / kPi) - 90) / 90);
    const double q2 = ap < 0 ? 0.0 : pow(ap, 0.25);
    if (index == 1) return sqrt(q1 * q2);
    double amin = 0, amax = 0;
#pragma unroll
    for (int i = 0; i < 4; i++) {
        const double a = fabs(ang[i]);
        amin = (i == 0 || a < amin) ? a : amin;
        amax = (i == 0 || a > amax) ? a : amax;
    }
    return sqrt(q1 * (amin / amax));
}

__global__ void __launch_bounds__(64)
k_quad_quality(int n, const double2 *__restrict__ quad_xy, int index, double *__restrict__ out)
{
    const int i = blockIdx.x * 64 + threadIdx.x;
    if (i >= n) return;
    P2 m[4];
#pragma unroll
    for (int k = 0; k < 4; k++) {
        const double2 v = quad_xy[(size_t)i * 4 + k];
        m[k] = mkp(v.x, v.y);
    }
    out[i] = quad_quality_index(m, index);
}

}
```

reinforcementlearning4meshgeneration_amd/csrc/meshenv_samples.h:

```cpp
#pragma once

#include "meshenv_smooth.h"

namespace meshenv {

constexpr int kSampMaxNeighbor = 3, kSampMaxRadius = 4, kSampSecMax = 32;

struct SampleParams {
    int n_neighbor, n_radius, index;
    double radius, quality_threshold;
};

enum { kSampOk = 0, kSampSkipped = 1, kSampLogOverflow = 2, kSampDegree = 3, kSampSectorOverflow = 4 };

__host__ __device__ __forceinline__ size_t samples_lds_bytes(int ring_cap, int log_cap)
{
    const size_t V = (size_t)ring_cap + log_cap;
    return V * sizeof(double2) + V * kSmoothMaxDeg * 2 + V + (size_t)log_cap + 64;
}

struct SampCtx {
    const double2 *coord;
    const unsigned short *adj;
    const unsigned char *deg;
// ... 30 lines not shown
    double amin = kInf, amax = -kInf;
    for (int i = 0; i < 4; i++) { const double a = fabs(ang[i]); amin = a < amin ? a : amin; amax = a > amax ? a : amax; }
    return sqrt(q1 * (amin / amax));
}

__device__ __forceinline__ int sample_sector(const SampCtx &s, int n_vert, int base, int start, int end_, int target, double radius,
                                             double start_angle, double end_angle, unsigned short *ids, P2 &syn, bool &overflow)
{
    const P2 pb = sp(s, base), ps = sp(s, start), pe = sp(s, end_);
    const double bl = radius * (0.5 * dist_lr(s.lr, pb, ps) + 0.5 * dist_lr(s.lr, pb, pe));
    double ds[kSampSecMax];
    int m = 0;
    for (int v = 0; v < n_vert; v++) {
        if (v == base) continue;
        const P2 pv = sp(s, v);
        const double d = dist_lr(s.lr, pb, pv);
        if (!(d <= bl) || v == start || v == end_ || v == target) continue;
        const double a = cw(pb, ps, pv);
        if (!(start_angle < a && a < end_angle)) continue;
        if (m == kSampSecMax) { overflow = true; continue; }
        int at = m;
        while (at > 0 && ds[at - 1] > d) { ds[at] = ds[at - 1]; ids[at] = ids[at - 1]; at--; }
        ds[at] = d; ids[at] = (unsigned short)v;
        m++;
    }
    const double a0 = cw(pb, ps, mkp(pb.x + 1, pb.y));
    const double mid = a0 - (start_angle + end_angle) / 2;
    syn = mkp(pb.x + bl * cos(mid), pb.y + bl * sin(mid));
    return m;
}

__device__ __forceinline__ bool sample_path(const SampCtx &s, int N, int root, int x0, int x1, int k, int *path)
{
    path[0] = root; path[1] = -1; path[2] = -1;
    if (N == 1) return k == 0;
    int seen = 0, ord1 = 0, a0 = -1;
    bool a0_dead = false;
    const int d0 = s.deg[root];
    for (int i = 0; i < d0; i++) {
        const int a = s.adj[(size_t)root * kSmoothMaxDeg + i];
        if (a == x0 || a == x1 || a == root) continue;
        if (N == 2) {
            if (seen == k) { path[1] = a; return true; }
            seen++;
            continue;
        }
        const bool quirk = ord1 == 1 && a0_dead;
        const int mid = quirk ? a0 : a, ex = quirk ? a0 : a;
        int kids = 0;
        const int d1 = s.deg[a];
        for (int j = 0; j < d1; j++) {
            const int b = s.adj[(size_t)a * kSmoothMaxDeg + j];
            if (b == x0 || b == x1 || b == root || b == ex) continue;
            kids++;
            if (seen == k) { path[1] = mid; path[2] = b; return true; }
            seen++;
        }
        if (ord1 == 0) { a0 = a; a0_dead = kids == 0; }
        ord1++;
    }
    return false;
}

__device__ __forceinline__ bool path_has(const int *path, int N, int v)
{
    return path[0] == v || (N > 1 && path[1] == v) || (N > 2 && path[2] == v);
}

template <bool kWrite>
__global__ void __launch_bounds__(64)
k_extract_samples(DevState S, int ring_cap, int which, const uint8_t *__restrict__ mask, SampleParams P, LibmRef lr,
                  long long *__restrict__ count_out, unsigned char *__restrict__ status_out, const long long *__restrict__ offsets,
                  double *__restrict__ samples, double *__restrict__ outputs, double *__restrict__ types)
{
    extern __shared__ double2 smem[];
    const int env = blockIdx.x, lane = lane_id();
    if (mask && mask[env] == 0) {
        if (lane == 0 && !kWrite) { count_out[env] = 0; status_out[env] = kSampSkipped; }
        return;
    }
    if (kWrite && (count_out[env] == 0 || status_out[env] != kSampOk)) return;
    const long long row_end = kWrite ? offsets[env + 1] : 0;
    const int log_cap = S.prm.log_cap;
    const EnvScalars sc = S.scal[env];
    const DevCold cold = load_cold(S);
    int n_elem = uniform_i32(sc.n_elem), n_new = uniform_i32(sc.n_new);
    int status = uniform_i32(sc.status), half = (status >> 4) & 1, overflow = status & kStLogOverflow;
    if (which) {
        const LastEpisode le = cold.last_ep[env];
        n_elem = uniform_i32(le.n_elem); n_new = uniform_i32(le.n_new);
        overflow = uniform_i32(le.flags) & 2;
        half ^= 1;
    }
    if (overflow || n_elem > log_cap || n_new > log_cap) {
        if (lane == 0 && !kWrite) { count_out[env] = 0; status_out[env] = kSampLogOverflow; }
        return;
    }
    const DomConst dc = S.dom[uniform_i32(sc.dom)];
    const int doff = uniform_i32(dc.off), n0 = uniform_i32(dc.n0), nv = n0 + n_new;
    const size_t lbase = ((size_t)env * 2 + half) * log_cap;
    const int4 *quads = reinterpret_cast<const int4 *>(cold.log_quads + lbase * 4);
    const double2 *vnew = cold.log_vxy + lbase;
    const int V = ring_cap + log_cap;
    double2 *coord = smem;
    unsigned short *adj = (unsigned short *)(coord + V);
    unsigned char *deg = (unsigned char *)(adj + (size_t)V * kSmoothMaxDeg);
    unsigned char *good = deg + V;
    for (int i = lane; i < n0; i += 64) coord[i] = cold.dom_xy[doff + i];
    for (int k = lane; k < n_new; k += 64) coord[n0 + k] = vnew[k];
    const bool too_many = build_segment_lists(quads, n_elem, n0, 0, nv, adj, deg, nullptr);
    if (__ballot(too_many) != 0ULL) {
        if (lane == 0 && !kWrite) { count_out[env] = 0; status_out[env] = kSampDegree; }
        return;
    }
    wave_sync();
    SampCtx s;
    s.coord = coord; s.adj = adj; s.deg = deg; s.lr = lr;
    auto vid = [&](int g) { return (g & kNewBit) ? n0 + (g & ~kNewBit) : g; };
    for (int e = lane; e < n_elem; e += 64) {
        const int4 q = quads[e];
        const int v[4] = {vid(q.x), vid(q.y), vid(q.z), vid(q.w)};
        good[e] = sample_element_quality(s, v, P.index) >= P.quality_threshold ? 1 : 0;
    }
    wave_sync();
    const int N = P.n_neighbor, R = P.n_radius;
    const int row = 2 * (2 * N + R);
    const double two_pi = 6.2832;
    long long base = kWrite ? offsets[env] : 0;
    long long total = 0;
    bool sector_overflow = false;
    const int items = 4 * n_elem;
    for (int it0 = 0; it0 < items; it0 += 64) {
        const int it = it0 + lane;
        const bool in = it < items;
        long long cnt = 0;
        int rp = 0, l_p = 0, r_p = 0, target = 0;
        int nR = 0, nL = 0, nRt = 0, nLt = 0;
        unsigned short sec[kSampMaxRadius][kSampSecMax];
        int sec_n[kSampMaxRadius] = {0, 0, 0, 0};
        P2 syn[kSampMaxRadius];
        long long fans = 1;
        bool live = false;
        if (in && good[it >> 2]) {
            live = true;
            const int4 q = quads[it >> 2];
            const int v[4] = {vid(q.x), vid(q.y), vid(q.z), vid(q.w)};
            const int i = it & 3;
            rp = v[i]; l_p = v[(i + 1) & 3]; r_p = v[(i + 3) & 3]; target = v[(i + 2) & 3];
            int path[3];
            for (int k = 0; sample_path(s, N, r_p, rp, l_p, k, path); k++) { nR++; nRt += path_has(path, N, target) ? 1 : 0; }
            for (int k = 0; sample_path(s, N, l_p, rp, r_p, k, path); k++) { nL++; nLt += path_has(path, N, target) ? 1 : 0; }
            const double angle = cw(sp(s, rp), sp(s, l_p), sp(s, r_p));
            for (int j = 1; j <= R; j++) {
                const double sa = ((double)(j - 1) * angle) / (double)R, ea = ((double)j * angle) / (double)R;
                sec_n[j - 1] = sample_sector(s, nv, rp, l_p, r_p, target, P.radius, sa, ea, sec[j - 1], syn[j - 1], sector_overflow);
                fans *= (long long)(sec_n[j - 1] + 1);
            }
            cnt = (long long)nR * fans * nL - (long long)nRt * fans * nLt;
        }
        long long incl = cnt;
        for (int o = 1; o < 64; o <<= 1) {
            const long long up = __shfl_up(incl, o, 64);
            if (lane >= o) incl += up;
        }
        const long long chunk_total = __shfl(incl, 63, 64);
        if (kWrite && live && cnt > 0) {
            long long at = base + total + (incl - cnt);
// ... 51 lines not shown
```

reinforcementlearning4meshgeneration_amd/csrc/meshenv_smooth.h:

```cpp
#pragma once

#include "meshenv_kernels.h"

namespace meshenv {

constexpr int kSmoothMaxDeg = 16;

enum { kSmoothSkipped = -1, kSmoothLogOverflow = -2, kSmoothDegree = -3, kSmoothNotFinished = -4, kSmoothIndexError = -5, kSmoothRaises = -6,
       kSmoothNonFinite = -7 };

__host__ __device__ __forceinline__ size_t smooth_lds_bytes(int ring_cap, int log_cap)
{
    return (size_t)(ring_cap + log_cap) * sizeof(double2) + (size_t)log_cap * (8 + kSmoothMaxDeg * 2 + 2 + 2) + 64;
}

__device__ __forceinline__ bool build_segment_lists(const int4 *__restrict__ quads, int n_elem, int n0, int first, int count,
                                                    unsigned short *adj, unsigned char *deg, unsigned char *n_mesh,
                                                    unsigned char *on_hole = nullptr)
{
    const int lane = lane_id();
    bool too_many = false;
    for (int r0 = 0; r0 < count; r0 += 64) {
        const int r = r0 + lane, u_me = first + r;
        const int me = u_me >= n0 ? (kNewBit | (u_me - n0)) : u_me;
        unsigned short mine[kSmoothMaxDeg] = {};
        unsigned long long uses = 0ULL;
        int d = 0, nm = 0;
        if (u_me < n0) {
            const int prev = u_me == 0 ? n0 - 1 : u_me - 1, next = u_me == n0 - 1 ? 0 : u_me + 1;
            mine[0] = (unsigned short)(u_me == n0 - 1 ? next : prev);
            mine[1] = (unsigned short)(u_me == n0 - 1 ? prev : next);
            d = 2;
            uses = 0x11ULL;
        }
        for (int e = 0; e < n_elem; e++) {
            const int4 q = quads[e];
            const int p = q.x == me ? 0 : (q.y == me ? 1 : (q.z == me ? 2 : (q.w == me ? 3 : -1)));
            if (p < 0 || r >= count) continue;
            nm += 1;
            const int first_g = p == 0 ? q.w : (p == 1 ? q.x : (p == 2 ? q.y : q.x));
            const int second_g = p == 0 ? q.y : (p == 1 ? q.z : (p == 2 ? q.w : q.z));
#pragma unroll
            for (int s = 0; s < 2; s++) {
                const int g = s == 0 ? first_g : second_g;
                const unsigned short u = (unsigned short)((g & kNewBit) ? n0 + (g & ~kNewBit) : g);
                int at = -1;
#pragma unroll
                for (int j = 0; j < kSmoothMaxDeg; j++) at = (at < 0 && j < d && mine[j] == u) ? j : at;
                if (at < 0) {
                    if (d < kSmoothMaxDeg) {
#pragma unroll
                        for (int j = 0; j < kSmoothMaxDeg; j++)
                            if (j == d) mine[j] = u;
                        at = d;
                        d += 1;
                    } else {
                        too_many = true;
                    }
                }
                if (at >= 0) uses += 1ULL << (4 * at);
            }
        }
        if (r < count) {
#pragma unroll
            for (int j = 0; j < kSmoothMaxDeg; j++) adj[(size_t)r * kSmoothMaxDeg + j] = mine[j];
            deg[r] = (unsigned char)d;
            if (n_mesh) n_mesh[r] = (unsigned char)(nm > 255 ? 255 : nm);
            if (on_hole) on_hole[r] = (uses & 0x1111111111111111ULL) != 0ULL ? 1 : 0;
        }
    }
    return too_many;
}

__global__ void __launch_bounds__(64)
k_smooth_interior(DevState S, int ring_cap, int which, const uint8_t *__restrict__ mask, const int32_t *__restrict__ gate,
                  int iteration, int32_t *__restrict__ sweeps_out, double *__restrict__ diff_out)
{
    extern __shared__ double2 smem[];
    const int env = blockIdx.x, lane = lane_id();
    if (mask && mask[env] == 0) {
        if (lane == 0 && sweeps_out) sweeps_out[env] = kSmoothSkipped;
        return;
    }
    if (gate && gate[env] < 0) {
        if (lane == 0 && sweeps_out) sweeps_out[env] = gate[env];
        return;
    }
    const int log_cap = S.prm.log_cap;
    const EnvScalars sc = S.scal[env];
    const DevCold cold = load_cold(S);
    int n = uniform_i32(sc.n), n_elem = uniform_i32(sc.n_elem), n_new = uniform_i32(sc.n_new);
    const int status = uniform_i32(sc.status);
    bool overflow = (status & kStLogOverflow) != 0;
    int half = (status >> 4) & 1;
    if (which) {
        const LastEpisode le = cold.last_ep[env];
        if (uniform_i32(le.episodes) <= 0) {
            if (lane == 0 && sweeps_out) sweeps_out[env] = kSmoothNotFinished;
            return;
        }
        n_elem = uniform_i32(le.n_elem); n_new = uniform_i32(le.n_new);
        overflow = (uniform_i32(le.flags) & 2) != 0;
        half ^= 1;
        n = 0;
    }
    if (overflow || n_elem > log_cap || n_new > log_cap) {
        if (lane == 0 && sweeps_out) sweeps_out[env] = kSmoothLogOverflow;
        return;
    }
    const DomConst dc = S.dom[uniform_i32(sc.dom)];
    const int doff = uniform_i32(dc.off), n0 = uniform_i32(dc.n0);
    const size_t lbase = ((size_t)env * 2 + half) * log_cap;
    const int4 *quads = reinterpret_cast<const int4 *>(cold.log_quads + lbase * 4);
    double2 *vnew = cold.log_vxy + lbase;

    double2 *coord = smem;
    double *xy_sum = (double *)(coord + ring_cap + log_cap);
    unsigned short *adj = (unsigned short *)(xy_sum + log_cap);
    unsigned short *lvl = adj + (size_t)log_cap * kSmoothMaxDeg;
    unsigned char *deg = (unsigned char *)(lvl + log_cap);
    unsigned char *front = deg + log_cap;

    for (int i = lane; i < n0; i += 64) coord[i] = cold.dom_xy[doff + i];
    for (int k = lane; k < n_new; k += 64) {
        coord[n0 + k] = vnew[k];
        front[k] = 0;
    }
    wave_sync();
    const int32_t *rid = S.ring_id + (size_t)env * S.cap;
    for (int i = lane; i < n; i += 64) {
        const int g = rid[i];
        if (g & kNewBit) front[g & ~kNewBit] = 1;
    }
    const bool too_many = build_segment_lists(quads, n_elem, n0, n0, n_new, adj, deg, nullptr, which ? front : nullptr);
    if (__ballot(too_many) != 0ULL) {
        if (lane == 0 && sweeps_out) sweeps_out[env] = kSmoothDegree;
        return;
    }
    wave_sync();
    for (int k = lane; k < n_new; k += 64) lvl[k] = (front[k] == 0 && deg[k] != 0) ? 1 : 0;
    wave_sync();
    for (int pass = 0; pass <= n_new; pass++) {
        bool changed = false;
        for (int k = lane; k < n_new; k += 64) {
            const int cur = lvl[k];
            if (cur == 0) continue;
            int m = 0;
            const int d = deg[k];
            for (int j = 0; j < d; j++) {
                const int u = (int)adj[(size_t)k * kSmoothMaxDeg + j] - n0;
                if (u >= 0 && u < k) { const int lu = lvl[u]; m = lu > m ? lu : m; }
            }
            if (m + 1 != cur) { lvl[k] = (unsigned short)(m + 1); changed = true; }
        }
        wave_sync();
        if (__ballot(changed) == 0ULL) break;
    }
    int my_max = 0;
    for (int k = lane; k < n_new; k += 64) my_max = lvl[k] > my_max ? lvl[k] : my_max;
    const int n_levels = wave_max_i32(my_max);
    double sum_coordinates = 0.0, diffs = 100.0;
    int it = 0;
    while (diffs > 0.001 && it < iteration) {
        it += 1;
        for (int l = 1; l <= n_levels; l++) {
            for (int k = lane; k < n_new; k += 64) {
                if (lvl[k] != l) continue;
                const int d = deg[k];
                const double2 v = coord[n0 + k];
                double x = 0.0, y = 0.0;
                for (int j = 0; j < d; j++) {
                    const double2 c = coord[adj[(size_t)k * kSmoothMaxDeg + j]];
                    x += c.x + v.x;
                    y += c.y + v.y;
                }
                const double nx = x / (double)(2 * d), ny = y / (double)(2 * d);
                coord[n0 + k] = make_double2(nx, ny);
                xy_sum[k] = nx + ny;
            }
            wave_sync();
        }
        double new_sum = 0.0;
        for (int k0 = 0; k0 < n_new; k0 += 64) {
            const int k = k0 + lane;
            const double sv = (k < n_new && lvl[k] != 0) ? xy_sum[k] : 0.0;
            const int m = n_new - k0 < 64 ? n_new - k0 : 64;
            for (int j = 0; j < m; j++) new_sum += lane_f64(sv, j);
        }
        diffs = fabs(new_sum - sum_coordinates);
        sum_coordinates = new_sum;
    }
    for (int k = lane; k < n_new; k += 64)
        if (front[k] == 0 && deg[k] != 0) vnew[k] = coord[n0 + k];
    if (lane == 0) {
        if (sweeps_out) sweeps_out[env] = it;
        if (diff_out) diff_out[env] = diffs;
    }
}


__host__ __device__ __forceinline__ size_t smooth_final_lds_bytes(int ring_cap, int log_cap)
{
    const size_t V = (size_t)ring_cap + log_cap;
    return V * sizeof(double2) + V * kSmoothMaxDeg * 2 + (size_t)ring_cap * 2 + V * 3 + 64;
}

struct SmoothGraph {
    const double2 *coord;
    const unsigned short *adj;
    const unsigned char *deg;
};

__device__ __forceinline__ bool graph_has(const SmoothGraph &g, int v, int w)
{
    const int d = uniform_i32((int)g.deg[v]);
    bool have = false;
    for (int j = 0; j < d; j++) have = have || (int)g.adj[(size_t)v * kSmoothMaxDeg + j] == w;
    return have;
}

__device__ __forceinline__ int nearest_common(const SmoothGraph &g, int a, int b, int skip, int point)
{
    const int da = uniform_i32((int)g.deg[a]);
    const double2 pp = g.coord[point];
    int best = -1;
    double bd = 0.0;
    for (int j = 0; j < da; j++) {
        const int w = uniform_i32((int)g.adj[(size_t)a * kSmoothMaxDeg + j]);
        if (w == skip || !graph_has(g, b, w)) continue;
        const double2 cw_ = g.coord[w];
        const double dd = dist(mkp(pp.x, pp.y), mkp(cw_.x, cw_.y));
        if (best < 0 || dd < bd) { best = w; bd = dd; }
    }
    return best;
}

__device__ __forceinline__ double2 estimate_4th_vertex(double2 origin, double2 left, double2 right, double factor,
                                                       bool has_suggest, double suggest_dist)
{
    const P2 o = mkp(origin.x, origin.y);
    double distance = (dist(o, mkp(left.x, left.y)) + dist(o, mkp(right.x, right.y))) * factor;
    if (has_suggest) {
        const double lim = 0.6 * suggest_dist;
        distance = lim < distance ? lim : distance;
    }
    const double r1x = (origin.x + origin.x) / 2, r1y = (origin.y + origin.y) / 2;
    const double r2x = (left.x + right.x) / 2, r2y = (left.y + right.y) / 2;
    const SinCos sc = sincos_nc(atan2_nc(r2y - r1y, r2x - r1x));
    return make_double2(r1x + distance * sc.c, r1y + distance * sc.s);
}

__global__ void __launch_bounds__(64)
k_smooth_final(DevState S, int ring_cap, int which, const uint8_t *__restrict__ mask, int iteration, double lr_1, double lr_2,
               int32_t *__restrict__ sweeps_out, double *__restrict__ diff_out)
{
    extern __shared__ double2 smem[];
    const int env = blockIdx.x, lane = lane_id();
    if (mask && mask[env] == 0) {
        if (lane == 0 && sweeps_out) sweeps_out[env] = kSmoothSkipped;
        return;
    }
    const int log_cap = S.prm.log_cap;
    const EnvScalars sc = S.scal[env];
    const DevCold cold = load_cold(S);
    int n = uniform_i32(sc.n), n_elem = uniform_i32(sc.n_elem), n_new = uniform_i32(sc.n_new);
    const int status = uniform_i32(sc.status);
    bool overflow = (status & kStLogOverflow) != 0, finished = n <= 5;
    int half = (status >> 4) & 1;
    if (which) {
        const LastEpisode le = cold.last_ep[env];
        n_elem = uniform_i32(le.n_elem); n_new = uniform_i32(le.n_new);
        overflow = (uniform_i32(le.flags) & 2) != 0;
        finished = uniform_i32(le.episodes) > 0 && (uniform_i32(le.flags) & 1) != 0;
        half ^= 1;
        n = 0;
    }
    if (overflow || n_elem > log_cap || n_new > log_cap || !finished) {
        if (lane == 0 && sweeps_out) sweeps_out[env] = !finished ? kSmoothNotFinished : kSmoothLogOverflow;
        return;
    }
    const DomConst dc = S.dom[uniform_i32(sc.dom)];
    const int doff = uniform_i32(dc.off), n0 = uniform_i32(dc.n0), nv = n0 + n_new;
    const size_t lbase = ((size_t)env * 2 + half) * log_cap;
    const int4 *quads = reinterpret_cast<const int4 *>(cold.log_quads + lbase * 4);
    double2 *vnew = cold.log_vxy + lbase;

    const int V = ring_cap + log_cap;
    double2 *coord = smem;
    unsigned short *adj = (unsigned short *)(coord + V);
    unsigned short *ringu = adj + (size_t)V * kSmoothMaxDeg;
    unsigned char *deg = (unsigned char *)(ringu + ring_cap);
    unsigned char *n_mesh = deg + V;
    unsigned char *front = n_mesh + V;

    for (int i = lane; i < n0; i += 64) coord[i] = cold.dom_xy[doff + i];
    for (int k = lane; k < n_new; k += 64) coord[n0 + k] = vnew[k];
    for (int u = lane; u < nv; u += 64) front[u] = 0;
    wave_sync();
    const int32_t *rid = S.ring_id + (size_t)env * S.cap;
    for (int i = lane; i < n; i += 64) {
        const int g = rid[i];
        const int u = (g & kNewBit) ? n0 + (g & ~kNewBit) : g;
        ringu[i] = (unsigned short)u;
        front[u] = 1;
    }
    const bool too_many = build_segment_lists(quads, n_elem, n0, 0, nv, adj, deg, n_mesh, which ? front : nullptr);
    if (__ballot(too_many) != 0ULL) {
        if (lane == 0 && sweeps_out) sweeps_out[env] = kSmoothDegree;
        return;
    }
    wave_sync();
    if (which) {
        int cnt = 0;
        for (int u0 = 0; u0 < nv; u0 += 64) {
            const int u = u0 + lane;
            const bool f = u < nv && front[u] != 0;
            const unsigned long long m = __ballot(f);
            if (f) {
                const int pos = cnt + __popcll(m & ((1ULL << lane) - 1ULL));
                if (pos < ring_cap) ringu[pos] = (unsigned short)u;
            }
            cnt += __popcll(m);
        }
        if (cnt == 0 && n_elem > 0) {
            const int4 q = quads[n_elem - 1];
            const int gq[4] = {q.x, q.y, q.z, q.w};
            if (lane < 4) {
                const int gg = lane == 0 ? gq[0] : (lane == 1 ? gq[1] : (lane == 2 ? gq[2] : gq[3]));
                const int u = (gg & kNewBit) ? n0 + (gg & ~kNewBit) : gg;
                ringu[lane] = (unsigned short)u;
                front[u] = 1;
            }
            cnt = 4;
        }
        n = cnt < ring_cap ? cnt : ring_cap;
        wave_sync();
    }
    SmoothGraph g;
    g.coord = coord; g.adj = adj; g.deg = deg;
    double sum_domain = 0.0;
    for (int i0 = 0; i0 < n0; i0 += 64) {
        const int i = i0 + lane;
        double sv = 0.0;
        if (i < n0) { const double2 c = coord[i]; sv = c.x + c.y; }
        const int m = n0 - i0 < 64 ? n0 - i0 : 64;
        for (int j = 0; j < m; j++) sum_domain += lane_f64(sv, j);
    }
    double sum_coordinates = 0.0, diffs = 100.0;
    int it = 0;
    bool index_error = false;
    while (!index_error && diffs > 0.001 && it < iteration) {
        it += 1;
        for (int k = n0; k < nv && !index_error; k++) {
            const int d = uniform_i32((int)deg[k]), nm = uniform_i32((int)n_mesh[k]);
            const unsigned short *row = adj + (size_t)k * kSmoothMaxDeg;
            bool pull = false;
            if (nm == 1) {
                if (d == 2) {
                    const int c0 = uniform_i32((int)row[0]), c1 = uniform_i32((int)row[1]);
                    const int origin = nearest_common(g, c0, c1, k, k);
                    if (origin < 0) { index_error = true; break; }
                    const double2 po = coord[origin];
                    double bd = kInf;
                    int bi = 0x7fffffff;
                    for (int i = lane; i < n; i += 64) {
                        const int w = ringu[i];
                        if (w == c0 || w == c1 || w == k || w == origin) continue;
                        const double2 pw = coord[w];
                        const double dd = dist(mkp(po.x, po.y), mkp(pw.x, pw.y));
                        if (dd < bd) { bd = dd; bi = i; }
                    }
                    const double dmin = wave_min_f64(bd);
                    const int imin = -wave_max_i32(bd == dmin && bi != 0x7fffffff ? -bi : INT32_MIN + 1);
                    if (imin != 0x7fffffff) {
                        const double2 nw = estimate_4th_vertex(po, coord[c0], coord[c1], 0.5, true, dmin);
                        if (lane == 0) coord[k] = nw;
                    }
                } else {
                    pull = true;
                }
            } else if (nm == 2) {
                int ub0 = -1, ub1 = -1, in0 = -1, nu = 0, ni = 0;
                for (int j = 0; j < d; j++) {
                    const int w = uniform_i32((int)row[j]);
                    if (uniform_i32((int)front[w]) != 0) { if (nu == 0) ub0 = w; else if (nu == 1) ub1 = w; nu += 1; }
                    else { if (ni == 0) in0 = w; ni += 1; }
                }
                if (ni == 1 && nu == 2) {
                    const int q1 = nearest_common(g, in0, ub0, k, k);
                    const int q2 = nearest_common(g, in0, ub1, k, k);
                    if (q1 < 0 || q2 < 0) { index_error = true; break; }
                    const double2 e1 = estimate_4th_vertex(coord[q1], coord[ub0], coord[in0], 0.7, false, 0.0);
                    const double2 e2 = estimate_4th_vertex(coord[q2], coord[ub1], coord[in0], 0.7, false, 0.0);
                    if (lane == 0) coord[k] = make_double2((e1.x + e2.x) / 2, (e1.y + e2.y) / 2);
                } else {
                    pull = true;
                }
            } else if (d != 0) {
                const double2 v = coord[k];
                double tx = 0.0, ty = 0.0;
                if (lane < d) {
                    const double2 c = coord[row[lane]];
                    tx = c.x + v.x;
                    ty = c.y + v.y;
                }
                double x = 0.0 + lane_f64(tx, 0), y = 0.0 + lane_f64(ty, 0);
                for (int j = 1; j < d; j++) {
                    x += lane_f64(tx, j);
                    y += lane_f64(ty, j);
                }
                if (lane == 0) coord[k] = make_double2(x / (double)(2 * d), y / (double)(2 * d));
            }
            if (pull) {
                const double lr = nm == 1 ? lr_1 : lr_2;
                double2 v = coord[k];
                for (int j = 0; j < d; j++) {
                    const double2 c = coord[uniform_i32((int)row[j])];
                    v.x = lr * v.x + (1 - lr) * c.x;
                    v.y = lr * v.y + (1 - lr) * c.y;
                }
                if (lane == 0) coord[k] = v;
            }
            wave_sync();
        }
        double new_sum = sum_domain;
        for (int k0 = 0; k0 < n_new; k0 += 64) {
            const int k = k0 + lane;
            double sv = 0.0;
            if (k < n_new) { const double2 c = coord[n0 + k]; sv = c.x + c.y; }
            const int m = n_new - k0 < 64 ? n_new - k0 : 64;
            for (int j = 0; j < m; j++) new_sum += lane_f64(sv, j);
        }
        diffs = fabs(new_sum - sum_coordinates);
        sum_coordinates = new_sum;
    }
    if (index_error) {
        if (lane == 0 && sweeps_out) sweeps_out[env] = kSmoothIndexError;
        return;
    }
    for (int k = lane; k < n_new; k += 64) vnew[k] = coord[n0 + k];
    if (!which) {
        double2 *rxy = S.ring_xy + (size_t)env * S.cap;
        for (int i = lane; i < n; i += 64) rxy[i] = coord[ringu[i]];
        if (lane == 0) S.scal[env].status = status & ~(kStRm1Bad | kStRp1Bad);
    }
    if (lane == 0) {
        if (sweeps_out) sweeps_out[env] = it;
        if (diff_out) diff_out[env] = diffs;
    }
}


struct FrontState {
    double2 *coord;
    const unsigned short *adj;
    const unsigned char *deg;
    const unsigned short *ringu;
    const double *tab;
    int n, n0;
    bool exact;
    int raised;
};

__device__ __forceinline__ P2 ldc(const FrontState &f, int v)
{
    const double2 c = f.coord[v];
    return mkp(c.x, c.y);
}

__device__ __forceinline__ double sq(const FrontState &f, double v) { return f.exact ? pow2_nc(v) : v * v; }
__device__ __forceinline__ double distf(const FrontState &f, P2 a, P2 b)
{
    return sqrt_pos(sq(f, a.x - b.x) + sq(f, a.y - b.y));
}

__device__ __forceinline__ double py_sqrt(FrontState &f, double v)
{
    if (v < 0) { f.raised = 1; return 0.0; }
    return sqrt(v);
}

__device__ __forceinline__ double py_div(FrontState &f, double a, double b, bool is_np)
{
    if (b == 0 && !is_np) { f.raised = 1; return 0.0; }
    return a / b;
}

__device__ __forceinline__ double deg2rad(double a) { return a * (kPi / 180.0); }
__device__ __forceinline__ double rad2deg(double a) { return a * (180.0 / kPi); }

__device__ __forceinline__ void circle_line(FrontState &f, double a, double b, double A, double B, double W, double dist_,
                                            bool np_A, P2 &v1, P2 &v2)
{
    if (B == 0) {
        const double wa = py_div(f, W, A, np_A);
        const double r = py_sqrt(f, sq(f, dist_) - sq(f, wa));
        v1 = mkp(wa + a, b + r);
        v2 = mkp(wa + a, b - r);
    } else if (A == 0) {
        const double wb = W / B;
        const double r = py_sqrt(f, sq(f, dist_) - sq(f, wb));
        v1 = mkp(a + r, wb + b);
        v2 = mkp(a - r, wb + b);
    } else {
        const double M = -A / B;
        const double N = (W + A * a + B * b) / B;
        const double t = 2 * M * b - 2 * M * N + 2 * a;
        const double m2 = sq(f, M);
        const double disc = fabs(sq(f, t) - 4 * (m2 + 1) * (sq(f, N - b) + sq(f, a) - sq(f, dist_)));
        const double den = 2 * (m2 + 1);
        const double sq = sqrt(disc);
        v1.x = (t + sq) / den;
        v2.x = (t - sq) / den;
        v1.y = M * v1.x + N;
        v2.y = M * v2.x + N;
    }
}

__device__ __forceinline__ P2 middle_vertex(const FrontState &f, P2 vertex, P2 left, P2 right, double tan_half)
{
    const P2 m = mkp((left.x + right.x) / 2, (left.y + right.y) / 2);
    const double A = right.x - left.x, B = right.y - left.y;
    const double D = distf(f, left, m) / tan_half;
    P2 v1, v2;
    if (B == 0) {
        v1 = mkp(m.x, m.y + D);
        v2 = mkp(m.x, m.y - D);
// ... 90 lines not shown
        }
    }
    wave_sync();
    return m;
}

__device__ __forceinline__ bool is_inside_boundary(const FrontState &f, P2 original, P2 moved, const unsigned short *b, int nb,
                                                   int left, int right)
{
    const int lane = lane_id();
    bool bad = false;
    if (lane < nb) {
        const int bi = b[lane], bp = b[lane == 0 ? nb - 1 : lane - 1];
        const bool skip = (left == bi || left == bp) && (right == bi || right == bp);
        if (!skip) bad = (cw(moved, ldc(f, bi), ldc(f, bp)) < kPi) != (cw(original, ldc(f, bi), ldc(f, bp)) < kPi);
    }
    return __ballot(bad) == 0ULL;
}

__device__ __forceinline__ P2 find_side_vertex(FrontState &f, int v, int _next, int next, int nn, double v_angle,
                                               unsigned short *cb)
{
    const P2 pv = ldc(f, v), pn = ldc(f, next), pnn = ldc(f, nn);
    const double d = (distf(f, pv, ldc(f, _next)) + distf(f, pv, pn) + distf(f, pn, pnn)) / 3;
    const bool np_A = next >= f.n0 || nn >= f.n0;
    double target = 45;
    for (int k = 0; k < 10; k++) {
        const P2 nv = side_vertex(f, pv, pn, pnn, f.tab[kFtCosSide + k], d, np_A);
        if (f.raised) return pv;
        if (target <= v_angle) return pv;
        const int nb = clockwise_vertices(f, v, cb);
        if (is_inside_boundary(f, pv, nv, cb, nb, _next, next)) return nv;
        target -= 5;
    }
    return pv;
}

__device__ __forceinline__ P2 find_indention_vertex(FrontState &f, int index, int q, unsigned short *cb)
{
    const int n = f.n, lane = lane_id();
    const int v = f.ringu[index], left = f.ringu[wrapi(index + 1, n)], right = f.ringu[wrapi(index - 1, n)];
    const int l2 = f.ringu[wrapi(index + 2, n)], r2 = f.ringu[wrapi(index - 2, n)];
    const P2 pv = ldc(f, v), pl = ldc(f, left), pr = ldc(f, right);
    const double d = (distf(f, pv, pl) + distf(f, pv, pr)) / 2;
    bool near = false, zero_div = false;
    for (int i = lane; i < n; i += 64) {
        const int w = f.ringu[i];
        if (!(w == v || w == r2 || w == right || w == left || w == l2)) near = near || distf(f, pv, ldc(f, w)) <= d;
        const int p1 = f.ringu[i == 0 ? n - 1 : i - 1], p2 = w;
        if (p1 != v && p2 != v) {
            const P2 a = ldc(f, p1), b = ldc(f, p2);
            const double A = b.x - a.x, B = b.y - a.y;
            const double den = sq(f, A) + sq(f, B);
            zero_div = zero_div || (den == 0 && p1 < f.n0 && p2 < f.n0);
            const double s = (A * pv.x + B * pv.y - B * a.y - A * a.x) / den;
            near = near || (0 <= s && s <= 1 && distf(f, pv, mkp(a.x + s * A, a.y + s * B)) <= d);
        }
    }
    if (__ballot(zero_div) != 0ULL) { f.raised = 1; return pv; }
    if (__ballot(near) == 0ULL) return pv;
    const double cos_a = f.tab[kFtCosInd + q];
    const bool np_A = v >= f.n0 || left >= f.n0;
    for (int times = 4; ; times++) {
        const P2 nv = indention_vertex(f, pv, pl, pr, cos_a, d / times, np_A);
        if (f.raised) return pv;
        if (times >= 10) return pv;
        const int nb = clockwise_vertices(f, v, cb);
        if (is_inside_boundary(f, pv, nv, cb, nb, left, right)) return nv;
    }
}

__global__ void __launch_bounds__(64)
k_smooth_front(DevState S, int ring_cap, const uint8_t *__restrict__ mask, int32_t *__restrict__ code_out,
               const double *__restrict__ tab, int libm_exact, double2 *__restrict__ nv_xy, const int32_t *__restrict__ nv_count,
               const int32_t *__restrict__ nv_gid)
{
    extern __shared__ double2 smem[];
    const int env = blockIdx.x, lane = lane_id();
    if (mask && mask[env] == 0) {
        if (lane == 0) code_out[env] = kSmoothSkipped;
        return;
    }
    const int log_cap = S.prm.log_cap;
    const EnvScalars sc = S.scal[env];
    const DevCold cold = load_cold(S);
    const int n = uniform_i32(sc.n), n_elem = uniform_i32(sc.n_elem), n_new = uniform_i32(sc.n_new);
    const int status = uniform_i32(sc.status);
    if ((status & kStLogOverflow) || n_elem > log_cap || n_new > log_cap) {
        if (lane == 0) code_out[env] = kSmoothLogOverflow;
        return;
    }
    const DomConst dc = S.dom[uniform_i32(sc.dom)];
    const int doff = uniform_i32(dc.off), n0 = uniform_i32(dc.n0), nv = n0 + n_new;
    const size_t lbase = ((size_t)env * 2 + ((status >> 4) & 1)) * log_cap;
    const int4 *quads = reinterpret_cast<const int4 *>(cold.log_quads + lbase * 4);
    double2 *vnew = cold.log_vxy + lbase;

    const int V = ring_cap + log_cap;
    double2 *coord = smem;
    unsigned short *adj = (unsigned short *)(coord + V);
    unsigned short *ringu = adj + (size_t)V * kSmoothMaxDeg;
    unsigned short *cb = ringu + ring_cap;
    unsigned char *deg = (unsigned char *)(cb + 2 * kSmoothMaxDeg);

    for (int i = lane; i < n0; i += 64) coord[i] = cold.dom_xy[doff + i];
    for (int k = lane; k < n_new; k += 64) coord[n0 + k] = vnew[k];
    const int32_t *rid = S.ring_id + (size_t)env * S.cap;
    for (int i = lane; i < n; i += 64) {
        const int g = rid[i];
        ringu[i] = (unsigned short)((g & kNewBit) ? n0 + (g & ~kNewBit) : g);
    }
    const bool too_many = build_segment_lists(quads, n_elem, n0, 0, nv, adj, deg, nullptr);
    if (__ballot(too_many) != 0ULL) {
        if (lane == 0) code_out[env] = kSmoothDegree;
        return;
    }
    wave_sync();
    FrontState f;
    f.coord = coord; f.adj = adj; f.deg = deg; f.ringu = ringu; f.n = n; f.n0 = n0; f.raised = 0; f.tab = tab; f.exact = libm_exact != 0;
    for (int i = 0; i < n && !f.raised; i++) {
        const int v = uniform_i32((int)ringu[i]);
        if (v < n0) continue;
        const int nxt = uniform_i32((int)ringu[i + 1 == n ? 0 : i + 1]), prv = uniform_i32((int)ringu[i == 0 ? n - 1 : i - 1]);
        const P2 pv = ldc(f, v), pn = ldc(f, nxt), pp = ldc(f, prv);
        const double v_rad = cw(pv, pn, pp);
        const double v_angle = rad2deg(v_rad);
        const int q = min(max(uniform_i32(angle_q(v_rad)), 0), kFtQ - 1);
        P2 nw = pv;
        if (v_angle <= 90) {
            double target = v_angle >= 45 ? v_angle : 45;
            const int row = v_angle >= 45 ? min(max(q, kFtMidQ0), kFtMidQ1) - kFtMidQ0 + 1 : 0;
            for (int k = 0; k < kFtMidSteps; k++) {
                const P2 cand = middle_vertex(f, pv, pn, pp, tab[kFtTanMid + row * kFtMidSteps + k]);
                if (target >= 135) break;
                const int nb = clockwise_vertices(f, v, cb);
                if (is_inside_boundary(f, pv, cand, cb, nb, nxt, prv)) { nw = cand; break; }
                target += 5;
            }
        } else if (v_angle <= 180) {
            const int nn_r = uniform_i32((int)ringu[wrapi(i - 2, n)]), nn_l = uniform_i32((int)ringu[wrapi(i + 2, n)]);
            const double left_angle = rad2deg(cw(pn, ldc(f, nn_l), pv));
            const double right_angle = rad2deg(cw(pp, pv, ldc(f, nn_r)));
            if (right_angle < 45) nw = find_side_vertex(f, v, nxt, prv, nn_r, right_angle, cb);
            else if (left_angle < 45) nw = find_side_vertex(f, v, prv, nxt, nn_l, left_angle, cb);
            else nw = find_indention_vertex(f, i, q, cb);
        } else if (v_angle <= 270) {
            nw = find_indention_vertex(f, i, q, cb);
        } else {
            const P2 m = mkp((pn.x + pp.x) / 2, (pn.y + pp.y) / 2);
            const double d = distf(f, m, pp) * tab[kFtTan45];
            const double A = pv.x - m.x, B = pv.y - m.y;
            const double qq = py_div(f, sq(f, d), sq(f, A) + sq(f, B), true);
            const double s = py_sqrt(f, qq);
            if (f.raised) break;
            const double ix = m.x + s * A, iy = m.y + s * B;
            if (!(isfinite(ix) && isfinite(iy))) { f.raised = 2; break; }
            if (lane == 0) coord[v] = make_double2(ix, iy);
            wave_sync();
            nw = find_indention_vertex(f, i, q, cb);
        }
        if (f.raised) break;
        if (!(isfinite(nw.x) && isfinite(nw.y))) { f.raised = 2; break; }
        if (lane == 0) coord[v] = make_double2(nw.x, nw.y);
        wave_sync();
    }
    double2 *rxy = S.ring_xy + (size_t)env * S.cap;
    for (int i = lane; i < n; i += 64) {
        const int u = ringu[i];
        if (u >= n0) {
            const double2 c = coord[u];
            vnew[u - n0] = c;
            rxy[i] = c;
        }
    }
    if (nv_xy) {
        const int n_nv = uniform_i32(nv_count[env]);
        for (int k = lane; k < n_nv; k += 64) {
            const int g = nv_gid[(size_t)env * ring_cap + k];
            if (g & kNewBit) nv_xy[(size_t)env * ring_cap + k] = coord[n0 + (g & ~kNewBit)];
        }
    }
    if (lane == 0) code_out[env] = f.raised == 2 ? kSmoothNonFinite : (f.raised ? kSmoothRaises : 0);
}

__host__ __device__ __forceinline__ size_t smooth_front_lds_bytes(int ring_cap, int log_cap)
{
    const size_t V = (size_t)ring_cap + log_cap;
    return V * sizeof(double2) + V * kSmoothMaxDeg * 2 + (size_t)ring_cap * 2 + 2 * kSmoothMaxDeg * 2 + V + 64;
}

struct alignas(32) Reselect {
    int32_t n_elem;
    int32_t ref;
    double bl, ct, st;
};

template <int kMode>
__global__ void __launch_bounds__(64)
k_rebuild_candidates(DevState S, int cap, const uint8_t *__restrict__ mask, const int32_t *__restrict__ sweeps,
                     Reselect *__restrict__ pend, float *__restrict__ pend_obs, float *__restrict__ obs_out, const LibmRef lr)
{
    extern __shared__ double2 smem[];
    const int env = blockIdx.x;
    if (mask && mask[env] == 0) return;
    if (sweeps && sweeps[env] < 0) return;
    Ctx c;
    c.tie = true;
    carve_lds(c, smem, cap);
    load_env(c, S, env);
    for (int i = c.lane; i < c.n; i += 64) {
        double cc, dd, k = 0.0;
        key_angle_terms(c, i, 0, cc, dd);
        const double a0 = cw_exact(cc, dd);
        key_angle_terms(c, i, 1, cc, dd);
        const double a1 = cw_exact(cc, dd);
        const bool ok = key_from_angles(S.prm, a0, a1, k);
        c.key[i] = k;
        c.stamp[i] = ok ? -i : kNotCand;
    }
    c.counter = 0;
    const int ref0 = c.ref, status0 = c.status;
    const double bl0 = c.bl, ct0 = c.ct, st0 = c.st;
    const float obs0 = c.obs;
    BqArgs bq;
    bq.skip = false;
    bq.mode = 0; bq.a = 0; bq.b = 0; bq.ang0 = 0; bq.ang1 = 0; bq.q_ang0 = 0; bq.q_ang2 = 0; bq.half01 = 0; bq.half23 = 0;
    find_next_state(c, S, bq, kMode == 2, nullptr, 0, lr);
    if (kMode == 0) {
        if (c.lane < kObsDim) pend_obs[(size_t)env * kObsDim + c.lane] = c.obs;
        if (c.lane == 0) {
            Reselect r;
            r.n_elem = c.n_elem; r.ref = c.ref; r.bl = c.bl; r.ct = c.ct; r.st = c.st;
            pend[env] = r;
        }
        c.ref = ref0; c.status = status0; c.bl = bl0; c.ct = ct0; c.st = st0; c.obs = obs0;
    } else {
        c.status &= ~(kStRm1Bad | kStRp1Bad);
        if (c.lane == 0) pend[env].n_elem = -1;
        if (obs_out && c.lane < kObsDim) obs_out[(size_t)env * kObsDim + c.lane] = c.obs;
    }
    c.ring_dirty = true;
    store_env(c, S);
}

__global__ void __launch_bounds__(64)
k_apply_reselect(DevState S, Reselect *__restrict__ pend, const float *__restrict__ pend_obs, float *__restrict__ obs_out)
{
    const int env = blockIdx.x, lane = lane_id();
    const Reselect r = pend[env];
    if (uniform_i32(r.n_elem) < 0) return;
    if (lane == 0) pend[env].n_elem = -1;
    EnvScalars *sc = S.scal + env;
    if (uniform_i32(sc->n_elem) != uniform_i32(r.n_elem)) return;
    if (lane < kObsDim) {
        const float o = pend_obs[(size_t)env * kObsDim + lane];
        S.obs_cache[(size_t)env * kObsDim + lane] = o;
        if (obs_out) obs_out[(size_t)env * kObsDim + lane] = o;
        if (S.msg) S.msg[(size_t)env * 21 + lane] = o;
    }
    if (lane == 0) {
        sc->ref = r.ref;
        sc->bl = r.bl; sc->ct = r.ct; sc->st = r.st;
        sc->status = (sc->status & ~(kStRm1Bad | kStRp1Bad | kStNoReference)) | (r.ref < 0 ? kStNoReference : 0);
    }
}


__global__ void k_move_mask(const uint8_t *__restrict__ code, uint8_t *__restrict__ mask, int n)
{
    const int e = blockIdx.x * blockDim.x + threadIdx.x;
    if (e < n) mask[e] = code[e] == (uint8_t)kMoveNeedsSmoothing ? 1 : 0;
}

__global__ void k_move_finish(DevState S, int cap, const uint8_t *__restrict__ mask, const int32_t *__restrict__ sweeps,
                              int32_t *__restrict__ nv_count, const int32_t *__restrict__ nv_gid, int32_t *__restrict__ nv_meta,
                              uint8_t *__restrict__ done, uint8_t *__restrict__ complete, uint8_t *__restrict__ code)
{
    const int e = blockIdx.x * blockDim.x + threadIdx.x;
    if (e >= S.n_envs || mask[e] == 0) return;
    const int sw = sweeps[e];
    if (sw == kSmoothRaises) {
        code[e] = (uint8_t)kMoveSmoothRaises;
        done[e] = 1;
        return;
    }
    int32_t *m = nv_meta + (size_t)e * kNvMeta;
    if (sw == kSmoothNonFinite) {
        const int cnt = nv_count[e];
        m[1] = cnt > 0 ? nv_gid[(size_t)e * cap] : 0; m[2] = cnt > 0 ? nv_gid[(size_t)e * cap + cnt - 1] : 0; m[3] = cnt; m[4] = m[0];
        nv_count[e] = 0;
        code[e] = (uint8_t)kMoveSmoothRaises;
        done[e] = 1;
        return;
    }
    if (sw < 0) return;
    const int cnt = nv_count[e], epoch = m[0];
    const int first = cnt > 0 ? nv_gid[(size_t)e * cap] : 0, last = cnt > 0 ? nv_gid[(size_t)e * cap + cnt - 1] : 0;
    bool dn = false;
    if (m[3] > 0 && cnt > 0) {
        dn = m[4] == epoch && first == m[1] && last == m[2] && cnt == m[3];
    }
    m[1] = first; m[2] = last; m[3] = cnt; m[4] = epoch;
    nv_count[e] = 0;
    const bool none = (S.scal[e].status & kStNoReference) != 0;
    done[e] = (uint8_t)((dn || none) ? 1 : 0);
    complete[e] = 0;
    code[e] = (uint8_t)(none ? kMoveNone : kMoveOk);
}

}
```

reinforcementlearning4meshgeneration_amd/csrc/meshenv_state.h:

```cpp
#pragma once

#include <hip/hip_runtime.h>
#include <stdint.h>

namespace meshenv {

constexpr int kObsDim = 18;
constexpr int kNotCand = INT32_MIN;

struct alignas(64) EnvScalars {
    int32_t n;
    int32_t ref;
    int32_t n_elem;
    int32_t n_new;
    int32_t counter;
    int32_t dom;
    int32_t failed;
    int32_t status;
    double bl;
    double area;
    double ct, st;
};

struct alignas(32) EnvCounters {
    unsigned long long last_change;
    unsigned long long valid, sum_n, sum_n_valid;
};

struct alignas(64) DomConst {
    double orig_area;
    double min_area;
    double crit_area;
    double bl;
    double ct, st;
    int32_t off;
    int32_t n0;
    int32_t ref;
    int32_t pad;
};

struct Params {
    double radius, max_ref_angle, w0, w1, min_degree, max_degree, same_eps, ray_length;
    int fail_limit, log_cap;
};

constexpr double kDefPi = 3.141592653589793;
constexpr double kDefRadius = 4.0, kDefMaxRefAngle = kDefPi * 0.972, kDefKeyLambda = 0.618;
constexpr double kDefMinDegree = 0.01 * kDefPi, kDefMaxDegree = 0.99 * kDefPi, kDefSameEps = 0.001, kDefRayLength = 10000.0;

__host__ __device__ inline void apply_default_params(Params &p)
{
    p.radius = kDefRadius; p.max_ref_angle = kDefMaxRefAngle; p.w0 = kDefKeyLambda; p.w1 = 1 - kDefKeyLambda;
    p.min_degree = kDefMinDegree; p.max_degree = kDefMaxDegree; p.same_eps = kDefSameEps; p.ray_length = kDefRayLength;
}

constexpr int kNewBit = 0x40000000;

struct LastEpisode {
    int32_t n_elem, n_new;
    int32_t flags;
    int32_t episodes;
};

struct DevCold {
    const double2 *dom_xy;
    double *dom_key;
    int32_t *dom_stamp;
    float *dom_obs;
    int32_t *log_quads;
    double2 *log_vxy;
    LastEpisode *last_ep;
    int64_t pad;
};

struct DevState {
    int n_domains;
    DomConst *dom;
    const DevCold *cold;
    int n_envs;
    int cap;
    double2 *ring_xy;
    int32_t *ring_id;
    double *ring_key;
    int32_t *ring_stamp;
    EnvScalars *scal;
    EnvCounters *cnt;
    float *obs_cache;
    float *msg;
#ifdef MESHENV_STAMPS
    unsigned long long *dbg;
#endif
    Params prm;
};

__device__ __forceinline__ DevCold load_cold(const DevState &S)
{
    const DevCold *p = S.cold;
    asm volatile("" : "+s"(p));
    return *p;
}

}
```

Baseline: 294.9 million.

## Pack per-env state into one contiguous block per environment

Replaces the separate structure-of-arrays buffers (scalars, counters, obs cache, ring xy/id/key/stamp) with a single per-env block at a 128-byte aligned stride, with each section at a fixed offset. Each wave's loads and stores for one env then land in a contiguous region, which should improve locality and cut the number of distinct base pointers and address computations. Host-side copies switch to strided 2D memcpy. The risk is that kernels which touch only one field across many envs, such as status or counter reads, now gather with a large stride.

Result: no change. 296.0 million (median of 3 runs) (+0.4%).

```diff
diff --git a/reinforcementlearning4meshgeneration_amd/csrc/meshenv_eval.h b/reinforcementlearning4meshgeneration_amd/csrc/meshenv_eval.h
--- a/reinforcementlearning4meshgeneration_amd/csrc/meshenv_eval.h
+++ b/reinforcementlearning4meshgeneration_amd/csrc/meshenv_eval.h
@@ -60,7 +60,7 @@
                     rec = true;
                     slot = A.offset[env] + cnt;
                     A.ep_env[slot] = env;
-                    A.ep_domain[slot] = S.scal[env].dom;
+                    A.ep_domain[slot] = env_scal(S, env)->dom;
                     A.ep_step[slot] = A.step;
                     A.ep_length[slot] = len;
                     A.ep_return[slot] = ret;
@@ -101,7 +101,7 @@
         todo &= todo - 1;
         if (k % kEvalWaves != wave) continue;
         double *row = A.ep_quality + (size_t)uniform_i32(s_slot[l]) * 4 * kQualityDim;
-        if ((scored >> l) & 1) env_quality(S, S.scal[base + l], cold, base + l, 1, nullptr, row, nullptr);
+        if ((scored >> l) & 1) env_quality(S, *env_scal(S, base + l), cold, base + l, 1, nullptr, row, nullptr);
         else if (lane < 4 * kQualityDim) row[lane] = 0.0;
     }
 }
diff --git a/reinforcementlearning4meshgeneration_amd/csrc/meshenv_hip.hip b/reinforcementlearning4meshgeneration_amd/csrc/meshenv_hip.hip
--- a/reinforcementlearning4meshgeneration_amd/csrc/meshenv_hip.hip
+++ b/reinforcementlearning4meshgeneration_amd/csrc/meshenv_hip.hip
@@ -516,8 +516,9 @@
     const int total_dom = dom_offsets_host[n_domains];
     h->dom_off_host.assign(dom_offsets_host, dom_offsets_host + n_domains + 1);
     h->env_dom_host.assign(env_domain_host, env_domain_host + n_envs);
-    const size_t total_env = (size_t)n_envs * (size_t)cap;
     S.cap = cap;
+    S.env_stride = EnvBlock::bytes(cap);
+    const size_t total_env = (size_t)n_envs * (size_t)S.env_stride;
 
     double2 *d_dom_xy = nullptr;
     DevCold &K = h->cold;
@@ -527,13 +528,7 @@
     CREATE_TRY(dev_alloc(h, &K.dom_key, (size_t)total_dom));
     CREATE_TRY(dev_alloc(h, &K.dom_stamp, (size_t)total_dom));
     CREATE_TRY(dev_alloc(h, &K.dom_obs, (size_t)n_domains * kObsDim));
-    CREATE_TRY(dev_alloc(h, &S.ring_xy, total_env));
-    CREATE_TRY(dev_alloc(h, &S.ring_id, total_env));
-    CREATE_TRY(dev_alloc(h, &S.ring_key, total_env));
-    CREATE_TRY(dev_alloc(h, &S.ring_stamp, total_env));
-    CREATE_TRY(dev_alloc(h, &S.scal, (size_t)n_envs));
-    CREATE_TRY(dev_alloc(h, &S.cnt, (size_t)n_envs));
-    CREATE_TRY(dev_alloc(h, &S.obs_cache, (size_t)n_envs * kObsDim));
+    CREATE_TRY(dev_alloc(h, &S.env_blocks, total_env));
     if (!h->env_lds_host.empty()) {
         CREATE_TRY(dev_alloc(h, &h->env_lds, (size_t)n_envs));
         CREATE_HIP(hipMemcpy(h->env_lds, h->env_lds_host.data(), sizeof(int2) * (size_t)n_envs, hipMemcpyHostToDevice));
@@ -595,11 +590,9 @@
             return MESHENV_E_STATE;
         }
     }
-    CREATE_HIP(hipMemcpy(S.scal, sc.data(), sizeof(EnvScalars) * (size_t)n_envs, hipMemcpyHostToDevice));
-    CREATE_HIP(hipMemset(S.ring_xy, 0, sizeof(double2) * total_env));
-    CREATE_HIP(hipMemset(S.ring_id, 0, sizeof(int32_t) * total_env));
-    CREATE_HIP(hipMemset(S.ring_key, 0, sizeof(double) * total_env));
-    CREATE_HIP(hipMemset(S.ring_stamp, 0, sizeof(int32_t) * total_env));
+    CREATE_HIP(hipMemsetAsync(S.env_blocks, 0, total_env, h->stream));
+    CREATE_HIP(hipMemcpy2DAsync(env_scal(S, 0), S.env_stride, sc.data(), sizeof(EnvScalars), sizeof(EnvScalars), (size_t)n_envs,
+                                hipMemcpyHostToDevice, h->stream));
 
     hipLaunchKernelGGL(k_init_domains, dim3(n_domains), dim3(64), lds, h->stream, S, cap);
     CREATE_HIP(hipGetLastError());
@@ -1193,7 +1186,7 @@
     HIP_TRY(h, hipMemcpy(&n, h->nv_count + env, sizeof(n), hipMemcpyDeviceToHost));
     HIP_TRY(h, hipMemcpy(meta, h->nv_meta + (size_t)env * kNvMeta, sizeof(meta), hipMemcpyDeviceToHost));
     EnvScalars s;
-    HIP_TRY(h, hipMemcpy(&s, h->S.scal + env, sizeof(s), hipMemcpyDeviceToHost));
+    HIP_TRY(h, hipMemcpy(&s, env_scal(h->S, env), sizeof(s), hipMemcpyDeviceToHost));
     const int n0 = h->dom_off_host[s.dom + 1] - h->dom_off_host[s.dom];
     auto gid = [n0](int32_t g) { return (g & kNewBit) ? n0 + (g & ~kNewBit) : g; };
     *count = n;
@@ -1298,7 +1291,7 @@
 __global__ void k_status(DevState S, uint8_t *out)
 {
     const int e = blockIdx.x * blockDim.x + threadIdx.x;
-    if (e < S.n_envs) out[e] = (uint8_t)(S.scal[e].status & 3);
+    if (e < S.n_envs) out[e] = (uint8_t)(env_scal(S, e)->status & 3);
 }
 
 int meshenv_get_status(MeshEnv *h, uint8_t *status_dev)
@@ -1321,21 +1314,20 @@
     MESHENV_ON_DEVICE(h);
     HIP_TRY(h, hipStreamSynchronize(h->stream));
     EnvScalars s;
-    HIP_TRY(h, hipMemcpy(&s, h->S.scal + env, sizeof(s), hipMemcpyDeviceToHost));
-    const size_t off = (size_t)env * (size_t)h->cap;
+    HIP_TRY(h, hipMemcpy(&s, env_scal(h->S, env), sizeof(s), hipMemcpyDeviceToHost));
     const int n0 = h->dom_off_host[s.dom + 1] - h->dom_off_host[s.dom];
     const int n = s.n;
     if (ring_ids_host) {
-        HIP_TRY(h, hipMemcpy(ring_ids_host, h->S.ring_id + off, sizeof(int32_t) * n, hipMemcpyDeviceToHost));
+        HIP_TRY(h, hipMemcpy(ring_ids_host, env_ring_id(h->S, env), sizeof(int32_t) * n, hipMemcpyDeviceToHost));
         for (int i = 0; i < n; i++)
             if (ring_ids_host[i] & kNewBit) ring_ids_host[i] = n0 + (ring_ids_host[i] & ~kNewBit);
     }
-    if (ring_xy_host) HIP_TRY(h, hipMemcpy(ring_xy_host, h->S.ring_xy + off, sizeof(double2) * n, hipMemcpyDeviceToHost));
+    if (ring_xy_host) HIP_TRY(h, hipMemcpy(ring_xy_host, env_ring_xy(h->S, env), sizeof(double2) * n, hipMemcpyDeviceToHost));
     if (cand_stamp_host || cand_key_host) {
         std::vector<int32_t> st((size_t)n);
         std::vector<double> ky((size_t)n);
-        HIP_TRY(h, hipMemcpy(st.data(), h->S.ring_stamp + off, sizeof(int32_t) * n, hipMemcpyDeviceToHost));
-        HIP_TRY(h, hipMemcpy(ky.data(), h->S.ring_key + off, sizeof(double) * n, hipMemcpyDeviceToHost));
+        HIP_TRY(h, hipMemcpy(st.data(), env_ring_stamp(h->S, env), sizeof(int32_t) * n, hipMemcpyDeviceToHost));
+        HIP_TRY(h, hipMemcpy(ky.data(), env_ring_key(h->S, env), sizeof(double) * n, hipMemcpyDeviceToHost));
         for (int i = 0; i < n; i++) {
             if (cand_stamp_host) cand_stamp_host[i] = st[i];
             if (cand_key_host) cand_key_host[i] = st[i] == kNotCand ? NAN : ky[i];
@@ -1375,7 +1367,7 @@
     MESHENV_ON_DEVICE(h);
     HIP_TRY(h, hipStreamSynchronize(h->stream));
     EnvScalars s;
-    HIP_TRY(h, hipMemcpy(&s, h->S.scal + env, sizeof(s), hipMemcpyDeviceToHost));
+    HIP_TRY(h, hipMemcpy(&s, env_scal(h->S, env), sizeof(s), hipMemcpyDeviceToHost));
     int half = (s.status >> 4) & 1, ne = s.n_elem, nnew = s.n_new;
     if (which) {
         LastEpisode le;
@@ -1457,8 +1449,11 @@
     HIP_TRY(h, hipStreamSynchronize(h->stream));
     std::vector<EnvCounters> c((size_t)h->n_envs);
     std::vector<EnvScalars> sc((size_t)h->n_envs);
-    HIP_TRY(h, hipMemcpy(c.data(), h->S.cnt, sizeof(EnvCounters) * (size_t)h->n_envs, hipMemcpyDeviceToHost));
-    HIP_TRY(h, hipMemcpy(sc.data(), h->S.scal, sizeof(EnvScalars) * (size_t)h->n_envs, hipMemcpyDeviceToHost));
+    HIP_TRY(h, hipMemcpy2DAsync(c.data(), sizeof(EnvCounters), env_cnt(h->S, 0), h->S.env_stride, sizeof(EnvCounters),
+                                (size_t)h->n_envs, hipMemcpyDeviceToHost, h->stream));
+    HIP_TRY(h, hipMemcpy2DAsync(sc.data(), sizeof(EnvScalars), env_scal(h->S, 0), h->S.env_stride, sizeof(EnvScalars),
+                                (size_t)h->n_envs, hipMemcpyDeviceToHost, h->stream));
+    HIP_TRY(h, hipStreamSynchronize(h->stream));
     uint64_t a = h->steps_done * (uint64_t)h->n_envs, b = 0, s = 0, sv = 0;
     for (int e = 0; e < h->n_envs; e++) {
         const EnvCounters &k = c[(size_t)e];
@@ -1478,7 +1473,8 @@
 {
     if (!h || !out_host) return MESHENV_E_ARG;
     HIP_TRY(h, hipStreamSynchronize(h->stream));
-    HIP_TRY(h, hipMemcpy(out_host, h->S.cnt, sizeof(EnvCounters) * (size_t)h->n_envs, hipMemcpyDeviceToHost));
+    HIP_TRY(h, hipMemcpy2D(out_host, sizeof(EnvCounters), env_cnt(h->S, 0), h->S.env_stride, sizeof(EnvCounters),
+                           (size_t)h->n_envs, hipMemcpyDeviceToHost));
     return MESHENV_OK;
 }
 int meshenv_debug_stamps(MeshEnv *h, uint64_t *out_host)
diff --git a/reinforcementlearning4meshgeneration_amd/csrc/meshenv_kernels.h b/reinforcementlearning4meshgeneration_amd/csrc/meshenv_kernels.h
--- a/reinforcementlearning4meshgeneration_amd/csrc/meshenv_kernels.h
+++ b/reinforcementlearning4meshgeneration_amd/csrc/meshenv_kernels.h
@@ -40,7 +40,7 @@
     int32_t *list;
     Scratch *sc;
     int lane, env;
-    size_t base;
+    char *blk;
     int n, ref, n_elem, failed, n_new, counter, status, dom;
     double bl, area, ct, st;
     bool ring_dirty;
@@ -102,39 +102,53 @@
     float obs;
 };
 
+struct RingOff {
+    unsigned key, id, stamp;
+};
+__device__ __forceinline__ RingOff ring_off(int cap)
+{
+    RingOff o;
+    o.key = EnvBlock::key(cap); o.id = EnvBlock::id(cap); o.stamp = EnvBlock::stamp(cap);
+    return o;
+}
+__device__ __forceinline__ double2 &g_xy(char *blk, unsigned i) { return *reinterpret_cast<double2 *>(blk + (EnvBlock::kRing + i * 16u)); }
+__device__ __forceinline__ double &g_key(char *blk, const RingOff &o, unsigned i) { return *reinterpret_cast<double *>(blk + (o.key + i * 8u)); }
+__device__ __forceinline__ int32_t &g_id(char *blk, const RingOff &o, unsigned i) { return *reinterpret_cast<int32_t *>(blk + (o.id + i * 4u)); }
+__device__ __forceinline__ int32_t &g_stamp(char *blk, const RingOff &o, unsigned i) { return *reinterpret_cast<int32_t *>(blk + (o.stamp + i * 4u)); }
+__device__ __forceinline__ float &g_obs(char *blk, unsigned lane) { return *reinterpret_cast<float *>(blk + (EnvBlock::kObs + lane * 4u)); }
+__device__ __forceinline__ EnvScalars &g_scal(char *blk) { return *reinterpret_cast<EnvScalars *>(blk + EnvBlock::kScal); }
+__device__ __forceinline__ EnvCounters &g_cnt(char *blk) { return *reinterpret_cast<EnvCounters *>(blk + EnvBlock::kCnt); }
+
 __device__ __forceinline__ EnvLoad load_env_issue(const DevState &S, int env, const bool with_keys = true)
 {
     EnvLoad L;
     const int lane = lane_id();
-    const size_t base = (size_t)env * S.cap;
-    L.s = S.scal[env];
+    char *blk = env_block(S, env);
+    const RingOff ro = ring_off(S.cap);
+    L.s = g_scal(blk);
     const int first = S.cap < 64 ? S.cap : 64;
-    const double2 *gxy = S.ring_xy + base;
-    const int32_t *gid = S.ring_id + base;
-    const double *gkey = S.ring_key + base;
-    const int32_t *gst = S.ring_stamp + base;
     const unsigned ul = (unsigned)lane;
     L.v_xy = make_double2(0, 0); L.w_xy = make_double2(0, 0);
     L.v_key = 0; L.w_key = 0;
     L.v_id = 0; L.v_st = kNotCand; L.w_id = 0; L.w_st = kNotCand;
     if (lane < first) {
-        L.v_xy = gxy[ul];
-        L.v_id = gid[ul];
+        L.v_xy = g_xy(blk, ul);
+        L.v_id = g_id(blk, ro, ul);
         if (with_keys) {
-            L.v_key = gkey[ul];
-            L.v_st = gst[ul];
+            L.v_key = g_key(blk, ro, ul);
+            L.v_st = g_stamp(blk, ro, ul);
         }
     }
     const bool second = S.cap > 64 && (int)(64u + ul) < S.cap;
     if (second) {
-        L.w_xy = gxy[64u + ul];
-        L.w_id = gid[64u + ul];
+        L.w_xy = g_xy(blk, 64u + ul);
+        L.w_id = g_id(blk, ro, 64u + ul);
         if (with_keys) {
-            L.w_key = gkey[64u + ul];
-            L.w_st = gst[64u + ul];
-        }
-    }
-    L.obs = lane < kObsDim ? S.obs_cache[(size_t)env * kObsDim + lane] : 0.0f;
+            L.w_key = g_key(blk, ro, 64u + ul);
+            L.w_st = g_stamp(blk, ro, 64u + ul);
+        }
+    }
+    L.obs = lane < kObsDim ? g_obs(blk, ul) : 0.0f;
     return L;
 }
 
@@ -144,14 +158,10 @@
     const int lane = lane_id();
     c.lane = lane;
     c.env = env;
-    c.base = (size_t)env * S.cap;
+    c.blk = env_block(S, env);
     const EnvScalars &s = L.s;
     const int lcap = lds_cap > 0 ? lds_cap : S.cap;
     const int first = lcap < 64 ? lcap : 64;
-    const double2 *gxy = S.ring_xy + c.base;
-    const int32_t *gid = S.ring_id + c.base;
-    const double *gkey = S.ring_key + c.base;
-    const int32_t *gst = S.ring_stamp + c.base;
     const unsigned ul = (unsigned)lane;
     const bool second = lcap > 64 && (int)(64u + ul) < lcap;
     c.obs = L.obs;
@@ -176,12 +186,15 @@
             c.stamp[64u + ul] = L.w_st;
         }
     }
-    for (unsigned i = 128u + ul; i < (unsigned)c.n; i += 64u) {
-        c.xy[i] = gxy[i];
-        c.id[i] = gid[i];
-        if (with_keys) {
-            c.key[i] = gkey[i];
-            c.stamp[i] = gst[i];
+    if (c.n > 128) {
+        const RingOff ro = ring_off(S.cap);
+        for (unsigned i = 128u + ul; i < (unsigned)c.n; i += 64u) {
+            c.xy[i] = g_xy(c.blk, i);
+            c.id[i] = g_id(c.blk, ro, i);
+            if (with_keys) {
+                c.key[i] = g_key(c.blk, ro, i);
+                c.stamp[i] = g_stamp(c.blk, ro, i);
+            }
         }
     }
     wave_sync();
@@ -195,35 +208,32 @@
 
 __device__ __forceinline__ void load_keys(Ctx &c, const DevState &S)
 {
-    const double *gkey = S.ring_key + c.base;
-    const int32_t *gst = S.ring_stamp + c.base;
+    const RingOff ro = ring_off(S.cap);
     for (unsigned i = (unsigned)c.lane; i < (unsigned)c.n; i += 64u) {
-        c.key[i] = gkey[i];
-        c.stamp[i] = gst[i];
-    }
-    wave_sync();
-}
-
-__device__ __forceinline__ void store_ring(const Ctx &c, const DevState &S)
-{
-    double2 *gxy = S.ring_xy + c.base;
-    int32_t *gid = S.ring_id + c.base;
-    double *gkey = S.ring_key + c.base;
-    int32_t *gst = S.ring_stamp + c.base;
+        c.key[i] = g_key(c.blk, ro, i);
+        c.stamp[i] = g_stamp(c.blk, ro, i);
+    }
+    wave_sync();
+}
+
+__device__ __forceinline__ void store_ring(const Ctx &c, char *blk, int cap)
+{
+    const RingOff ro = ring_off(cap);
     for (unsigned i = (unsigned)c.lane; i < (unsigned)c.n; i += 64u) {
-        gxy[i] = c.xy[i];
-        gid[i] = c.id[i];
-        gkey[i] = c.key[i];
-        gst[i] = c.stamp[i];
+        g_xy(blk, i) = c.xy[i];
+        g_id(blk, ro, i) = c.id[i];
+        g_key(blk, ro, i) = c.key[i];
+        g_stamp(blk, ro, i) = c.stamp[i];
     }
 }
 
 __device__ __forceinline__ void store_env(Ctx &c, const DevState &S, bool ring_elsewhere = false)
 {
     wave_sync();
+    char *blk = c.blk;
     if (c.ring_dirty) {
-        if (!ring_elsewhere) store_ring(c, S);
-        if (c.lane < kObsDim) S.obs_cache[(size_t)c.env * kObsDim + c.lane] = c.obs;
+        if (!ring_elsewhere) store_ring(c, blk, S.cap);
+        if (c.lane < kObsDim) g_obs(blk, (unsigned)c.lane) = c.obs;
     }
     if (c.lane == 0) {
         if (c.ring_dirty) {
@@ -231,9 +241,9 @@
             s.n = c.n; s.ref = c.ref; s.n_elem = c.n_elem; s.failed = c.failed; s.n_new = c.n_new;
             s.counter = c.counter; s.status = c.status; s.dom = c.dom; s.bl = c.bl; s.area = c.area;
             s.ct = c.ct; s.st = c.st;
-            S.scal[c.env] = s;
+            g_scal(blk) = s;
         } else {
-            int2 *fs = reinterpret_cast<int2 *>(&S.scal[c.env].failed);
+            int2 *fs = reinterpret_cast<int2 *>(&g_scal(blk).failed);
             *fs = make_int2(c.failed, c.status);
         }
     }
@@ -1388,7 +1398,7 @@
     const int d = blockIdx.x;
     c.lane = lane_id();
     c.env = -1;
-    c.base = 0;
+    c.blk = nullptr;
     c.dom = d;
     const DomConst dc = S.dom[d];
     const DevCold cold = load_cold(S);
@@ -1441,19 +1451,19 @@
     const bool doit = mask == nullptr || mask[env] != 0;
     c.lane = lane_id();
     if (!doit) {
-        if (obs_out && c.lane < kObsDim) obs_out[(size_t)env * kObsDim + c.lane] = S.obs_cache[(size_t)env * kObsDim + c.lane];
+        if (obs_out && c.lane < kObsDim) obs_out[(size_t)env * kObsDim + c.lane] = env_obs_cache(S, env)[c.lane];
         return;
     }
     c.env = env;
-    c.base = (size_t)env * S.cap;
-    c.dom = uniform_i32(S.scal[env].dom);
+    c.blk = env_block(S, env);
+    c.dom = uniform_i32(g_scal(c.blk).dom);
     if (first) {
         c.n = 0; c.n_elem = 0; c.n_new = 0; c.status = 0;
     } else {
-        c.n = uniform_i32(S.scal[env].n);
-        c.n_elem = uniform_i32(S.scal[env].n_elem);
-        c.n_new = uniform_i32(S.scal[env].n_new);
-        c.status = uniform_i32(S.scal[env].status);
+        c.n = uniform_i32(g_scal(c.blk).n);
+        c.n_elem = uniform_i32(g_scal(c.blk).n_elem);
+        c.n_new = uniform_i32(g_scal(c.blk).n_new);
+        c.status = uniform_i32(g_scal(c.blk).status);
     }
     const int n_old = c.n;
     reset_from_domain(c, S);
@@ -1467,11 +1477,11 @@
         if (first) {
             z.last_change = 0; z.valid = 0; z.sum_n = 0; z.sum_n_valid = 0;
         } else {
-            z = S.cnt[env];
+            z = g_cnt(c.blk);
             z.sum_n += (unsigned long long)n_old * (step_now - z.last_change);
             z.last_change = step_now;
         }
-        S.cnt[env] = z;
+        g_cnt(c.blk) = z;
     }
     store_env(c, S);
     if (obs_out && c.lane < kObsDim) obs_out[(size_t)env * kObsDim + c.lane] = c.obs;
@@ -1534,9 +1544,10 @@
     const unsigned long long stamp_c0 = __builtin_amdgcn_s_memtime();
 #endif
     if (!kMulti && (auto_reset & 2)) {
-        const EnvScalars s0 = S.scal[env];
+        char *blk0 = env_block(S, env);
+        const EnvScalars s0 = g_scal(blk0);
         const int lane0 = lane_id();
-        const float ob = lane0 < kObsDim ? S.obs_cache[(size_t)env * kObsDim + lane0] : 0.0f;
+        const float ob = lane0 < kObsDim ? g_obs(blk0, (unsigned)lane0) : 0.0f;
         const int st0 = uniform_i32(s0.status), failed0 = uniform_i32(s0.failed) + 1, ne0 = uniform_i32(s0.n_elem);
         const bool memo = (a0 <= -0.5f && (st0 & kStRm1Bad) != 0) || (a0 >= 0.5f && (st0 & kStRp1Bad) != 0);
         if (memo && uniform_i32(s0.ref) >= 0 && uniform_i32(s0.n) > 5 && failed0 < S.prm.fail_limit) {
@@ -1548,7 +1559,7 @@
                 reward[env] = rw;
                 done[env] = 0;
                 complete[env] = 1;
-                S.scal[env].failed = failed0;
+                g_scal(blk0).failed = failed0;
             }
             return;
         }
@@ -1558,7 +1569,7 @@
 #ifndef MESHENV_STAMPS
     EnvCounters cnt0;
     cnt0.last_change = 0; cnt0.valid = 0; cnt0.sum_n = 0; cnt0.sum_n_valid = 0;
-    if (kMulti) cnt0 = S.cnt[env];
+    if (kMulti) cnt0 = *env_cnt(S, env);
 #endif
     if (light) load_env(c, S, env, false);
     else load_env(c, S, env);
@@ -1598,7 +1609,7 @@
             const KStepArgs L = late_kstep_args<kDefaultParams>();
             const bool l_auto = (L.auto_reset & 1) != 0;
             if (r.valid || (r.done && l_auto)) {
-                k = L.S.cnt[env];
+                k = g_cnt(c.blk);
                 const unsigned long long next = L.step0 + 1ULL;
                 k.sum_n += (unsigned long long)n_before * (next - k.last_change);
                 k.last_change = next;
@@ -1620,7 +1631,7 @@
                 L.S.msg[(size_t)env * 21 + c.lane] = v;
             }
             store_env(c, L.S);
-            if (k_dirty && c.lane == 0) L.S.cnt[env] = k;
+            if (k_dirty && c.lane == 0) g_cnt(c.blk) = k;
             return;
         }
 #endif
@@ -1662,7 +1673,7 @@
             L.S.msg[(size_t)env * 21 + c.lane] = v;
         }
         store_env(c, L.S);
-        if (k_dirty && c.lane == 0) L.S.cnt[env] = k;
+        if (k_dirty && c.lane == 0) g_cnt(c.blk) = k;
         return;
     }
 #endif
@@ -1677,13 +1688,13 @@
         EnvCounters k;
         k.last_change = stamp_t0; k.valid = stamp_t1; k.sum_n = __builtin_amdgcn_s_memrealtime();
         k.sum_n_valid = st_valid | ((unsigned long long)(a0 <= -0.5f ? 1 : (a0 >= 0.5f ? 2 : 0)) << 8);
-        S.cnt[env] = k;
+        g_cnt(c.blk) = k;
     }
     if (c.lane == 0) c.sc->stamps[15] = __builtin_amdgcn_s_memtime() - stamp_c0;
     wave_sync();
     if (c.lane < 16) S.dbg[(size_t)env * 16 + c.lane] = c.sc->stamps[c.lane];
 #else
-    if (k_dirty && c.lane == 0) S.cnt[env] = k;
+    if (k_dirty && c.lane == 0) g_cnt(c.blk) = k;
 #endif
 }
 
@@ -1833,6 +1844,7 @@
     const StepResult r = env_finish(c, S_in.prm, d);
     const int env = c.env;
     const DevState S = late_state(S_in);
+    c.blk = env_block(S, env);
     const StepOuts o = late_outs();
     float *__restrict__ obs_out = o.obs_out;
     double *__restrict__ reward = o.reward;
@@ -1863,11 +1875,11 @@
     }
     store_env(c, S, has_helper && !r.done);
     if ((r.valid || (r.done && auto_reset)) && c.lane == 0) {
-        EnvCounters k = cnt_late ? S.cnt[env] : cnt0;
+        EnvCounters k = cnt_late ? g_cnt(c.blk) : cnt0;
         k.sum_n += (unsigned long long)n_before * (step0 + 1ULL - k.last_change);
         k.last_change = step0 + 1ULL;
         if (r.valid) { k.valid += 1ULL; k.sum_n_valid += (unsigned long long)n_before; }
-        S.cnt[env] = k;
+        g_cnt(c.blk) = k;
     }
 }
 
@@ -2009,9 +2021,8 @@
         const double rew = reward_on_helper(c, S, d, uniform_i32(h.n), uniform_i32(h.dom), &h.upd_done);
         wave_sync();
         if (c.n > 5) {
-            c.env = henv;
-            c.base = (size_t)henv * S.cap;
-            store_ring(c, late_state(S));
+            const DevState SL = late_state(S);
+            store_ring(c, env_block(SL, henv), SL.cap);
         }
         if (c.lane == 0) {
             *(volatile int *)&h.helper_done = 1;
@@ -2028,7 +2039,7 @@
     else carve_lds(c, (char *)smem + (size_t)src * env_bytes, cap);
     c.lane = tid & 63;
     c.env = uniform_i32(h.env);
-    c.base = (size_t)c.env * S.cap;
+    c.blk = env_block(late_state(S), c.env);
     c.n = uniform_i32(h.n); c.ref = uniform_i32(h.ref); c.n_elem = uniform_i32(h.n_elem); c.failed = uniform_i32(h.failed);
     if (kSmall) __builtin_assume(c.n <= 64 && c.n >= 0);
     c.n_new = uniform_i32(h.n_new); c.counter = uniform_i32(h.counter); c.status = uniform_i32(h.status); c.dom = uniform_i32(h.dom);
@@ -2041,7 +2052,7 @@
     d.p0 = uniform_i32(d.p0); d.p1 = uniform_i32(d.p1); d.p2 = uniform_i32(d.p2); d.p3 = uniform_i32(d.p3);
     d.t0 = uniform_i32(d.t0); d.t1 = uniform_i32(d.t1); d.lo = uniform_i32(d.lo); d.hi = uniform_i32(d.hi);
     d.ok = 1;
-    const EnvCounters cnt0 = S.cnt[c.env];
+    const EnvCounters cnt0 = g_cnt(c.blk);
     const int n_before = c.n;
     env_apply(c, S, d, helpers ? &h.upd_done : nullptr);
 #ifdef MESHENV_STAMPS
diff --git a/reinforcementlearning4meshgeneration_amd/csrc/meshenv_quality.h b/reinforcementlearning4meshgeneration_amd/csrc/meshenv_quality.h
--- a/reinforcementlearning4meshgeneration_amd/csrc/meshenv_quality.h
+++ b/reinforcementlearning4meshgeneration_amd/csrc/meshenv_quality.h
@@ -147,7 +147,7 @@
                   int32_t *__restrict__ count_out)
 {
     const int env = blockIdx.x;
-    const EnvScalars sc = S.scal[env];
+    const EnvScalars sc = *env_scal(S, env);
     const DevCold cold = load_cold(S);
     env_quality(S, sc, cold, env, which, elem_out, stats_out ? stats_out + (size_t)env * 4 * kQualityDim : nullptr,
                 count_out ? count_out + env : nullptr);
diff --git a/reinforcementlearning4meshgeneration_amd/csrc/meshenv_samples.h b/reinforcementlearning4meshgeneration_amd/csrc/meshenv_samples.h
--- a/reinforcementlearning4meshgeneration_amd/csrc/meshenv_samples.h
+++ b/reinforcementlearning4meshgeneration_amd/csrc/meshenv_samples.h
@@ -136,7 +136,7 @@
     if (kWrite && (count_out[env] == 0 || status_out[env] != kSampOk)) return;
     const long long row_end = kWrite ? offsets[env + 1] : 0;
     const int log_cap = S.prm.log_cap;
-    const EnvScalars sc = S.scal[env];
+    const EnvScalars sc = *env_scal(S, env);
     const DevCold cold = load_cold(S);
     int n_elem = uniform_i32(sc.n_elem), n_new = uniform_i32(sc.n_new);
     int status = uniform_i32(sc.status), half = (status >> 4) & 1, overflow = status & kStLogOverflow;
diff --git a/reinforcementlearning4meshgeneration_amd/csrc/meshenv_smooth.h b/reinforcementlearning4meshgeneration_amd/csrc/meshenv_smooth.h
--- a/reinforcementlearning4meshgeneration_amd/csrc/meshenv_smooth.h
+++ b/reinforcementlearning4meshgeneration_amd/csrc/meshenv_smooth.h
@@ -87,7 +87,7 @@
         return;
     }
     const int log_cap = S.prm.log_cap;
-    const EnvScalars sc = S.scal[env];
+    const EnvScalars sc = *env_scal(S, env);
     const DevCold cold = load_cold(S);
     int n = uniform_i32(sc.n), n_elem = uniform_i32(sc.n_elem), n_new = uniform_i32(sc.n_new);
     const int status = uniform_i32(sc.status);
@@ -127,7 +127,7 @@
         front[k] = 0;
     }
     wave_sync();
-    const int32_t *rid = S.ring_id + (size_t)env * S.cap;
+    const int32_t *rid = env_ring_id(S, env);
     for (int i = lane; i < n; i += 64) {
         const int g = rid[i];
         if (g & kNewBit) front[g & ~kNewBit] = 1;
@@ -261,7 +261,7 @@
         return;
     }
     const int log_cap = S.prm.log_cap;
-    const EnvScalars sc = S.scal[env];
+    const EnvScalars sc = *env_scal(S, env);
     const DevCold cold = load_cold(S);
     int n = uniform_i32(sc.n), n_elem = uniform_i32(sc.n_elem), n_new = uniform_i32(sc.n_new);
     const int status = uniform_i32(sc.status);
@@ -297,7 +297,7 @@
     for (int k = lane; k < n_new; k += 64) coord[n0 + k] = vnew[k];
     for (int u = lane; u < nv; u += 64) front[u] = 0;
     wave_sync();
-    const int32_t *rid = S.ring_id + (size_t)env * S.cap;
+    const int32_t *rid = env_ring_id(S, env);
     for (int i = lane; i < n; i += 64) {
         const int g = rid[i];
         const int u = (g & kNewBit) ? n0 + (g & ~kNewBit) : g;
@@ -440,9 +440,9 @@
     }
     for (int k = lane; k < n_new; k += 64) vnew[k] = coord[n0 + k];
     if (!which) {
-        double2 *rxy = S.ring_xy + (size_t)env * S.cap;
+        double2 *rxy = env_ring_xy(S, env);
         for (int i = lane; i < n; i += 64) rxy[i] = coord[ringu[i]];
-        if (lane == 0) S.scal[env].status = status & ~(kStRm1Bad | kStRp1Bad);
+        if (lane == 0) env_scal(S, env)->status = status & ~(kStRm1Bad | kStRp1Bad);
     }
     if (lane == 0) {
         if (sweeps_out) sweeps_out[env] = it;
@@ -699,7 +699,7 @@
         return;
     }
     const int log_cap = S.prm.log_cap;
-    const EnvScalars sc = S.scal[env];
+    const EnvScalars sc = *env_scal(S, env);
     const DevCold cold = load_cold(S);
     const int n = uniform_i32(sc.n), n_elem = uniform_i32(sc.n_elem), n_new = uniform_i32(sc.n_new);
     const int status = uniform_i32(sc.status);
@@ -722,7 +722,7 @@
 
     for (int i = lane; i < n0; i += 64) coord[i] = cold.dom_xy[doff + i];
     for (int k = lane; k < n_new; k += 64) coord[n0 + k] = vnew[k];
-    const int32_t *rid = S.ring_id + (size_t)env * S.cap;
+    const int32_t *rid = env_ring_id(S, env);
     for (int i = lane; i < n; i += 64) {
         const int g = rid[i];
         ringu[i] = (unsigned short)((g & kNewBit) ? n0 + (g & ~kNewBit) : g);
@@ -781,7 +781,7 @@
         if (lane == 0) coord[v] = make_double2(nw.x, nw.y);
         wave_sync();
     }
-    double2 *rxy = S.ring_xy + (size_t)env * S.cap;
+    double2 *rxy = env_ring_xy(S, env);
     for (int i = lane; i < n; i += 64) {
         const int u = ringu[i];
         if (u >= n0) {
@@ -867,11 +867,11 @@
     const Reselect r = pend[env];
     if (uniform_i32(r.n_elem) < 0) return;
     if (lane == 0) pend[env].n_elem = -1;
-    EnvScalars *sc = S.scal + env;
+    EnvScalars *sc = env_scal(S, env);
     if (uniform_i32(sc->n_elem) != uniform_i32(r.n_elem)) return;
     if (lane < kObsDim) {
         const float o = pend_obs[(size_t)env * kObsDim + lane];
-        S.obs_cache[(size_t)env * kObsDim + lane] = o;
+        env_obs_cache(S, env)[lane] = o;
         if (obs_out) obs_out[(size_t)env * kObsDim + lane] = o;
         if (S.msg) S.msg[(size_t)env * 21 + lane] = o;
     }
@@ -919,7 +919,7 @@
     }
     m[1] = first; m[2] = last; m[3] = cnt; m[4] = epoch;
     nv_count[e] = 0;
-    const bool none = (S.scal[e].status & kStNoReference) != 0;
+    const bool none = (env_scal(S, e)->status & kStNoReference) != 0;
     done[e] = (uint8_t)((dn || none) ? 1 : 0);
     complete[e] = 0;
     code[e] = (uint8_t)(none ? kMoveNone : kMoveOk);
diff --git a/reinforcementlearning4meshgeneration_amd/csrc/meshenv_state.h b/reinforcementlearning4meshgeneration_amd/csrc/meshenv_state.h
--- a/reinforcementlearning4meshgeneration_amd/csrc/meshenv_state.h
+++ b/reinforcementlearning4meshgeneration_amd/csrc/meshenv_state.h
@@ -62,6 +62,30 @@
     int32_t episodes;
 };
 
+struct EnvBlock {
+    static constexpr unsigned kScal = 0;
+    static constexpr unsigned kCnt = 64;
+#ifndef X_OBS
+#define X_OBS 96
+#define X_RING 192
+#endif
+    static constexpr unsigned kObs = X_OBS;
+    static constexpr unsigned kRing = X_RING;
+    __host__ __device__ static constexpr unsigned key(int cap) { return kRing + 16u * (unsigned)cap; }
+    __host__ __device__ static constexpr unsigned id(int cap) { return kRing + 24u * (unsigned)cap; }
+    __host__ __device__ static constexpr unsigned stamp(int cap) { return kRing + 28u * (unsigned)cap; }
+    __host__ __device__ static constexpr unsigned bytes(int cap) { return (kRing + 32u * (unsigned)cap + 127u) / 128u * 128u; }
+};
+static_assert(EnvBlock::kCnt == EnvBlock::kScal + sizeof(EnvScalars), "counters follow the record");
+static_assert(EnvBlock::kObs >= EnvBlock::kCnt + sizeof(EnvCounters), "the cached observation follows the counters");
+static_assert(EnvBlock::kObs + kObsDim * sizeof(float) <= EnvBlock::kRing, "the observation fits its padded section");
+static_assert(EnvBlock::kScal % alignof(EnvScalars) == 0 && EnvBlock::kCnt % alignof(EnvCounters) == 0, "section alignment");
+static_assert(EnvBlock::kRing % 64 == 0, "ring sections start on a 64-byte sector (cap is a multiple of 16)");
+static_assert(EnvBlock::key(16) % 16 == 0 && EnvBlock::id(16) % 16 == 0 && EnvBlock::stamp(16) % 16 == 0, "16-byte sections");
+static_assert(EnvBlock::bytes(16) == 768 && EnvBlock::bytes(32) == 1280 && EnvBlock::bytes(64) == 2304, "block sizes");
+static_assert(EnvBlock::bytes(16) % 128 == 0 && EnvBlock::bytes(48) % 128 == 0 && EnvBlock::bytes(80) % 128 == 0 &&
+              EnvBlock::bytes(640) % 128 == 0, "the stride is a multiple of 128 B");
+
 struct DevCold {
     const double2 *dom_xy;
     double *dom_key;
@@ -79,13 +103,8 @@
     const DevCold *cold;
     int n_envs;
     int cap;
-    double2 *ring_xy;
-    int32_t *ring_id;
-    double *ring_key;
-    int32_t *ring_stamp;
-    EnvScalars *scal;
-    EnvCounters *cnt;
-    float *obs_cache;
+    unsigned env_stride;
+    char *env_blocks;
     float *msg;
 #ifdef MESHENV_STAMPS
     unsigned long long *dbg;
@@ -100,4 +119,37 @@
     return *p;
 }
 
+__host__ __device__ __forceinline__ char *env_block(const DevState &S, int env)
+{
+    return S.env_blocks + (size_t)env * S.env_stride;
 }
+__host__ __device__ __forceinline__ EnvScalars *env_scal(const DevState &S, int env)
+{
+    return reinterpret_cast<EnvScalars *>(env_block(S, env) + EnvBlock::kScal);
+}
+__host__ __device__ __forceinline__ EnvCounters *env_cnt(const DevState &S, int env)
+{
+    return reinterpret_cast<EnvCounters *>(env_block(S, env) + EnvBlock::kCnt);
+}
+__host__ __device__ __forceinline__ float *env_obs_cache(const DevState &S, int env)
+{
+    return reinterpret_cast<float *>(env_block(S, env) + EnvBlock::kObs);
+}
+__host__ __device__ __forceinline__ double2 *env_ring_xy(const DevState &S, int env)
+{
+    return reinterpret_cast<double2 *>(env_block(S, env) + EnvBlock::kRing);
+}
+__host__ __device__ __forceinline__ double *env_ring_key(const DevState &S, int env)
+{
+    return reinterpret_cast<double *>(env_block(S, env) + EnvBlock::key(S.cap));
+}
+__host__ __device__ __forceinline__ int32_t *env_ring_id(const DevState &S, int env)
+{
+    return reinterpret_cast<int32_t *>(env_block(S, env) + EnvBlock::id(S.cap));
+}
+__host__ __device__ __forceinline__ int32_t *env_ring_stamp(const DevState &S, int env)
+{
+    return reinterpret_cast<int32_t *>(env_block(S, env) + EnvBlock::stamp(S.cap));
+}
+
+}
```
